# fu5ha/rayn

Measured on AMD Instinct MI355X. Metric: Mpath-samples/sec, higher is better.
Workload: dtype f32; 1 GPU; 1920x1080, 1024 spp, 8 bounces, MandelBox SDF + homogeneous volume [BASELINE configs[2]]; fma_policy=unfused (reference default build), parallelism=tiles round-robin over 1 GPU(s), build_variant=product, resolve_kernel=k_resolve_blk<128, 8>

## Files before the change

### include/rayn_hip.h

```cpp
#ifndef RAYN_HIP_H
#define RAYN_HIP_H

#include <stddef.h>
#include <stdint.h>

#ifdef __cplusplus
extern "C" {
#endif

#define RAYN_MAX_HITABLES 16
#define RAYN_MAX_MATERIALS 16
#define RAYN_MAX_LIGHTS 16
#define RAYN_FIS_TABLE_SIZE 512
#define RAYN_FILM_FLOATS_PER_PIXEL 10

typedef enum {
    RAYN_OK = 0,
    RAYN_ERR_INVALID_ARG = -1,
    RAYN_ERR_NO_DEVICE = -2,
    RAYN_ERR_HIP = -3,
    RAYN_ERR_NO_WORLD = -4,
    RAYN_ERR_OOM = -5
} rayn_status;

// ... 258 lines not shown
                            const uint32_t* d_low_object, const void* d_high_records, const uint32_t* d_high_object, float* d_out_color,
                            float* d_out_alpha, float* d_out_background, float* d_out_normal, float* d_out_weight, void* hip_stream);

typedef struct { uint32_t confidence;  } rayn_temporal_upscale_params;
int rayn_hip_temporal_upscale_device(rayn_ctx* ctx, const rayn_frame_params* p, const rayn_upscale_params* up, const rayn_temporal_params* tp,
                                     const rayn_temporal_upscale_params* sp, const rayn_camera* low_camera, const rayn_camera* prev_camera,
                                     float prev_time_start, const float* d_color, const float* d_alpha, const float* d_background,
                                     const float* d_normal, const void* d_low_records, const uint32_t* d_low_object, const void* d_high_records,
                                     const uint32_t* d_high_object, const void* d_prev_history, void* d_new_history, size_t history_bytes,
                                     float* d_out_color, float* d_out_alpha, float* d_out_background, float* d_out_normal, float* d_out_weight,
                                     void* hip_stream);

typedef struct {
    uint32_t samples;
    float radius;
    float ambient;
} rayn_preview_params;
size_t rayn_preview_scratch_bytes(uint32_t width, uint32_t height, uint32_t samples);
int rayn_hip_preview_device(rayn_ctx* ctx, const rayn_frame_params* p, const rayn_preview_params* pp, const float* d_samples,
                            const float* d_scramble, float* d_out_color, float* d_out_alpha, float* d_out_normal, float* d_out_ao,
                            void* d_out_records, uint32_t* d_out_object, void* d_scratch, size_t scratch_bytes, void* hip_stream);

typedef struct {
    float depth_tolerance;
} rayn_interpolate_params;
typedef struct {
    const float* d_color;
    const float* d_alpha;
    const float* d_background;
    const float* d_normal;
    const void* d_records;
    const uint32_t* d_object;
    const rayn_camera* camera;
    float time_start;
} rayn_interpolate_key;
int rayn_hip_interpolate_device(rayn_ctx* ctx, const rayn_frame_params* p, const rayn_interpolate_params* ip, const rayn_interpolate_key* key_a,
                                const rayn_interpolate_key* key_b, const void* d_gbuffer_records, const uint32_t* d_gbuffer_object,
                                float* d_out_color, float* d_out_alpha, float* d_out_background, float* d_out_normal, uint32_t* d_out_source,
                                void* hip_stream);

size_t rayn_png_stream_bound(uint32_t width, uint32_t height, uint32_t bpp);
size_t rayn_png_scratch_bytes(uint32_t width, uint32_t height, uint32_t bpp);
int rayn_hip_png_encode_device(rayn_ctx* ctx, uint32_t width, uint32_t height, uint32_t bpp, const uint8_t* d_img, void* d_out, size_t out_bytes,
                               void* d_scratch, size_t scratch_bytes, void* hip_stream);

size_t rayn_png_scratch_bytes_lz77(uint32_t width, uint32_t height, uint32_t bpp);
int rayn_hip_png_encode_lz77_device(rayn_ctx* ctx, uint32_t width, uint32_t height, uint32_t bpp, const uint8_t* d_img, void* d_out, size_t out_bytes,
                                    void* d_scratch, size_t scratch_bytes, void* hip_stream);
size_t rayn_deflate_stream_bound(size_t n);
size_t rayn_deflate_scratch_bytes(size_t n);
int rayn_hip_deflate_lz77_device(rayn_ctx* ctx, const void* d_data, size_t n, uint32_t stride, void* d_out, size_t out_bytes, void* d_scratch,
                                 size_t scratch_bytes, void* hip_stream);

size_t rayn_exr_stream_bound(uint32_t width, uint32_t height, uint32_t n_channels, const uint32_t* layout);
size_t rayn_exr_scratch_bytes(uint32_t width, uint32_t height, uint32_t n_channels, const uint32_t* layout, uint32_t matches);
int rayn_hip_exr_encode_device(rayn_ctx* ctx, uint32_t width, uint32_t height, uint32_t n_channels, const void* const* d_planes,
                               const uint32_t* layout, uint32_t matches, void* d_out, size_t out_bytes, void* d_scratch, size_t scratch_bytes,
                               void* hip_stream);

size_t rayn_jpeg_scan_bound(uint32_t width, uint32_t height, uint32_t bpp, uint32_t subsampling, uint32_t restart_interval);
size_t rayn_jpeg_scratch_bytes(uint32_t width, uint32_t height, uint32_t bpp, uint32_t subsampling, uint32_t restart_interval);
int rayn_jpeg_quant_table(uint32_t quality, uint32_t which, uint8_t* out);
int rayn_jpeg_huffman_table(uint32_t which, uint8_t* bits, uint8_t* vals, uint32_t n);
int rayn_hip_jpeg_encode_device(rayn_ctx* ctx, uint32_t width, uint32_t height, uint32_t bpp, uint32_t quality, uint32_t subsampling,
                                uint32_t restart_interval, const uint8_t* d_img, void* d_out, size_t out_bytes, void* d_scratch,
                                size_t scratch_bytes, void* hip_stream);

uint32_t rayn_sets_1d(uint32_t max_bounces, uint32_t volume_marches);
uint32_t rayn_sets_2d(uint32_t max_bounces, uint32_t volume_marches);
int rayn_build_rd_tables(uint32_t spp, uint32_t sets_1d, uint32_t sets_2d, uint64_t frame,
                         float* samples_1d, float* samples_2d);
int rayn_build_scramble(uint32_t width, uint32_t height, float* scramble);
enum { RAYN_FILTER_BLACKMAN_HARRIS = 0, RAYN_FILTER_BOX = 1, RAYN_FILTER_MITCHELL = 2, RAYN_FILTER_LANCZOS = 3 };
int rayn_build_fis_table(uint32_t filter_kind, float radius, float* table512);
int rayn_build_fis_table_ex(uint32_t filter_kind, float radius, float param0, float param1,
                            float* table512);
uint32_t rayn_tile_count(uint32_t width, uint32_t height, uint32_t tile_w, uint32_t tile_h);

int rayn_hip_set_profiling(rayn_ctx* ctx, int timing, int count_evals);
int rayn_hip_get_eval_counts(const rayn_ctx* ctx, uint64_t out[3]);
int rayn_hip_get_sdf_iterations(const rayn_ctx* ctx, uint64_t out[3]);
int rayn_hip_get_elision_counts(const rayn_ctx* ctx, uint64_t out[3]);
int rayn_hip_get_stage_slots(const rayn_ctx* ctx, uint64_t out[2]);
int rayn_hip_set_workers(rayn_ctx* ctx, int n_workers, uint64_t min_paths);
int rayn_hip_set_batch_paths(rayn_ctx* ctx, uint64_t paths);
int rayn_hip_set_cold_bytes(rayn_ctx* ctx, uint64_t bytes);
int rayn_hip_fma_policy(void);
int rayn_hip_set_fma_policy(rayn_ctx* ctx, int policy);
size_t rayn_hip_sizeof(int which);
const char* rayn_hip_build_variant(void);

int rayn_hip_set_tile_subset(rayn_ctx* ctx, const uint32_t* tiles, uint32_t n);

int rayn_hip_set_trace_tile(rayn_ctx* ctx, int tile_index);
int64_t rayn_hip_get_trace(const rayn_ctx* ctx, uint32_t* out, uint64_t cap_records);

int rayn_hip_probe_huffman(rayn_ctx* ctx, uint32_t n_symbols, uint32_t n_sets, const uint32_t* counts,
                           uint32_t* out_clen, uint32_t* out_tab);
int rayn_hip_probe_jpeg_transform(rayn_ctx* ctx, uint32_t width, uint32_t height, uint32_t bpp, uint32_t quality, uint32_t subsampling,
                                  const uint8_t* img, int16_t* out_coef);
int rayn_hip_probe_jpeg_entropy(rayn_ctx* ctx, uint32_t width, uint32_t height, uint32_t bpp, uint32_t subsampling, uint32_t restart_interval,
                                const int16_t* coef, uint32_t fill_byte, uint8_t* out, size_t out_bytes);
int rayn_hip_probe_shade_limits(const rayn_ctx* ctx, uint32_t* stream_blocks, uint32_t* list_ids_per_block,
                                uint32_t* setup_threads);
int rayn_hip_probe_shade(rayn_ctx* ctx, const rayn_frame_params* p, const float* samples_1d, const float* samples_2d,
                         const float* scramble, const float* fis_table, uint32_t depth, uint32_t n_slots,
                         uint32_t max_slots, uint32_t nee_cap, const uint32_t* ref, uint32_t n_pool,
                         const float* geo0, const float* geo1, const float* col0, const float* col1,
                         uint32_t sentinel, float* out_geo0, float* out_geo1, float* out_col0, float* out_col1,
                         float* out_aov, uint32_t* out_term_key, uint8_t* out_term_info,
                         uint64_t* out_alive_mask, uint8_t* out_bgrp_cnt, uint64_t* out_jobs);
int rayn_hip_probe_raygen(rayn_ctx* ctx, const rayn_frame_params* p, const float* samples_1d, uint64_t n_samples_1d,
                          const float* samples_2d, uint64_t n_samples_2d, const float* scramble, uint64_t n_scramble,
                          const float* fis_table, uint32_t n_tiles, const uint32_t* tiles, uint32_t n_pool,
                          uint32_t surplus, uint32_t sentinel, float* out_geo0, float* out_geo1, float* out_col0,
                          float* out_col1, float* out_aov, uint32_t* out_term_key, uint8_t* out_term_info,
                          uint32_t* out_q, uint32_t* out_pgrp_tile, uint32_t* out_tgb, uint32_t* out_tgc,
                          uint32_t* out_ctl, float* out_records);
int rayn_hip_probe_march_limits(const rayn_ctx* ctx, uint32_t* chunk, uint32_t* endgame_entries,
                                uint32_t* persistent_blocks, uint32_t* bulb_rays);
int rayn_hip_probe_sdf_dist(rayn_ctx* ctx, const rayn_frame_params* p, uint32_t hitable_index,
                            const float* pts_xyz, float* out, uint32_t n);
int rayn_hip_probe_sdf_dist_as(rayn_ctx* ctx, const rayn_frame_params* p, uint32_t hitable_index, int32_t sdfk,
                               uint32_t fast_div, float t0, const float* pts_xyz, float* out, uint32_t n);
int rayn_hip_probe_scene_dispatch(rayn_ctx* ctx, const rayn_frame_params* p, int32_t* out);
int rayn_hip_probe_extend(rayn_ctx* ctx, const rayn_frame_params* p, uint32_t depth,
                          const float* org_xyz, const float* dir_xyz, float* out_t,
                          uint32_t* out_obj, uint32_t n);
int rayn_hip_probe_shadow(rayn_ctx* ctx, const rayn_frame_params* p, const float* start_xyz,
                          const float* end_xyz, float* out, uint32_t n);
int rayn_hip_probe_detmath(rayn_ctx* ctx, uint32_t op, const float* a, const float* b, float* out,
                           uint32_t n);
int rayn_hip_probe_shading(rayn_ctx* ctx, const rayn_frame_params* p, uint32_t op, uint32_t index,
                           const float* in, float* out, const float* aux, uint32_t n);
int rayn_hip_probe_queue(rayn_ctx* ctx, uint32_t nclass, uint32_t n_tiles, const uint32_t* tile_groups,
                         const uint32_t* q, const uint8_t* ent_obj, const uint8_t* survive, uint32_t n_refs,
                         uint32_t cap_groups_bin, uint32_t cap_groups_repack, uint32_t max_entries,
                         uint32_t max_slots, uint32_t sentinel, uint32_t out_slots, uint32_t* out_bq,
                         uint32_t* out_qn, uint32_t* out_tile, uint32_t* out_cls_cnt,
                         uint32_t* out_cls_base, uint64_t* ctl_io);
int rayn_hip_probe_resolve(rayn_ctx* ctx, uint32_t width, uint32_t spp, uint32_t n_tiles, const uint32_t* tiles,
                           uint32_t max_tile_pixels, uint32_t n_paths, const uint8_t* term_info,
                           const uint32_t* term_key, const float* col0_rgb, const float* aov_xyz,
                           const uint32_t* aov_obj, const uint32_t* base_hist, uint32_t hist_stride,
                           uint32_t n_depths, uint32_t sentinel, uint32_t out_pixels, float* out_color,
                           float* out_alpha, float* out_background, float* out_normal);

#ifdef __cplusplus
}
#endif
#endif
```

### rayn_amd/_lib.py

```python
import ctypes as C
import os
import subprocess

from . import _abi


class RaynHipError(RuntimeError):
    pass


_CSRC = os.path.join(os.path.dirname(os.path.abspath(__file__)), "csrc")
DEFAULT_LIB_PATH = os.path.join(_CSRC, "librayn_hip.so")


def _lib_path():
    alt = os.environ.get("RAYN_HIP_LIB")
    if not alt:
        return DEFAULT_LIB_PATH
    if os.environ.get("RAYN_HIP_ALLOW_VARIANT") != "1":
        raise RaynHipError(f"RAYN_HIP_LIB={alt} is set but RAYN_HIP_ALLOW_VARIANT=1 is not: refusing to load a non-product build of librayn_hip.so")
    return alt



EXPORTS = [
    "rayn_hip_create", "rayn_hip_create_multi", "rayn_hip_device_count", "rayn_hip_table_broadcasts", "rayn_hip_destroy", "rayn_hip_last_error", "rayn_hip_upload_world", "rayn_hip_render_frame",
    "rayn_hip_render_frame_device", "rayn_hip_get_stats", "rayn_sets_1d", "rayn_sets_2d", "rayn_build_rd_tables",
    "rayn_build_scramble", "rayn_build_fis_table", "rayn_build_fis_table_ex", "rayn_tile_count", "rayn_hip_set_profiling", "rayn_hip_get_eval_counts",
    "rayn_hip_set_batch_paths", "rayn_hip_set_cold_bytes", "rayn_hip_set_workers", "rayn_hip_set_tile_subset", "rayn_hip_set_trace_tile", "rayn_hip_get_trace", "rayn_hip_fma_policy", "rayn_hip_set_fma_policy", "rayn_hip_sizeof", "rayn_hip_probe_sdf_dist",
    "rayn_hip_probe_extend", "rayn_hip_probe_shadow", "rayn_hip_probe_detmath", "rayn_hip_probe_shading", "rayn_hip_probe_queue", "rayn_hip_probe_resolve", "rayn_hip_probe_march_limits", "rayn_hip_probe_shade", "rayn_hip_probe_shade_limits", "rayn_hip_probe_raygen", "rayn_hip_probe_sdf_dist_as", "rayn_hip_probe_scene_dispatch", "rayn_hip_probe_huffman", "rayn_hip_probe_jpeg_transform", "rayn_hip_probe_jpeg_entropy", "rayn_hip_build_variant",
    "rayn_hip_get_entry_stats", "rayn_hip_get_sdf_iterations", "rayn_hip_get_elision_counts", "rayn_hip_get_stage_slots", "rayn_share_pixels", "rayn_hip_render_frame_packed_device", "rayn_hip_unpack_share_device",
    "rayn_save_to_bpp", "rayn_hip_save_to_pixels_device", "rayn_denoise_scratch_bytes", "rayn_hip_denoise_device",
    "rayn_progressive_seed", "rayn_progressive_state_bytes", "rayn_hip_progressive_reset_device", "rayn_hip_progressive_accumulate_device",
    "rayn_hip_progressive_fetch_active", "rayn_hip_progressive_tile_report",
    "rayn_denoise_variance_scratch_bytes", "rayn_hip_denoise_variance_device",
    "rayn_gbuffer_scratch_bytes", "rayn_hip_gbuffer_device", "rayn_temporal_history_bytes", "rayn_hip_temporal_accumulate_device",
    "rayn_temporal_moments_bytes", "rayn_hip_temporal_accumulate_moments_device", "rayn_hip_denoise_temporal_variance_device",
    "rayn_hip_denoise_temporal_variance_feedback_device", "rayn_hip_temporal_accumulate_resample_device",
    "rayn_display_scratch_bytes", "rayn_hip_display_pixels_device", "rayn_hip_display_color_device",
    "rayn_hip_upscale_device", "rayn_hip_temporal_upscale_device",
    "rayn_preview_scratch_bytes", "rayn_hip_preview_device",
    "rayn_hip_interpolate_device",
    "rayn_png_stream_bound", "rayn_png_scratch_bytes", "rayn_hip_png_encode_device",
    "rayn_png_scratch_bytes_lz77", "rayn_hip_png_encode_lz77_device",
    "rayn_deflate_stream_bound", "rayn_deflate_scratch_bytes", "rayn_hip_deflate_lz77_device",
    "rayn_exr_stream_bound", "rayn_exr_scratch_bytes", "rayn_hip_exr_encode_device",
    "rayn_jpeg_scan_bound", "rayn_jpeg_scratch_bytes", "rayn_jpeg_quant_table", "rayn_jpeg_huffman_table", "rayn_hip_jpeg_encode_device",
]


def build(force=False):
    if force:
        subprocess.check_call(["make", "-C", _CSRC, "clean"], stdout=subprocess.DEVNULL)
    subprocess.check_call(["make", "-C", _CSRC], stdout=subprocess.DEVNULL)


_lib = None


def lib():
    global _lib
    if _lib is None:
        LIB_PATH = _lib_path()
        if not os.path.exists(LIB_PATH):
            raise RaynHipError(f"{LIB_PATH} is missing: run `python -c 'import __graft_entry__ as g; g.build()'` "
                               "(there is no CPU fallback)")
        try:
            import torch
        except ImportError:
            pass
        L = C.CDLL(LIB_PATH)
        fp, up, vp = C.POINTER(C.c_float), C.POINTER(C.c_uint32), C.c_void_p
        L.rayn_hip_create.argtypes = [C.c_int, C.POINTER(vp)]
        L.rayn_hip_create_multi.argtypes = [C.POINTER(C.c_int), C.c_int, C.POINTER(vp)]
        L.rayn_hip_device_count.argtypes = [vp]
        L.rayn_hip_table_broadcasts.argtypes = [vp]
        L.rayn_hip_table_broadcasts.restype = C.c_uint64
        L.rayn_hip_destroy.argtypes = [vp]
        L.rayn_hip_destroy.restype = None
        L.rayn_hip_last_error.argtypes = [vp]
        L.rayn_hip_last_error.restype = C.c_char_p
        L.rayn_hip_upload_world.argtypes = [vp, C.POINTER(_abi.WorldDesc)]
        L.rayn_hip_render_frame.argtypes = [vp, C.POINTER(_abi.FrameParams), fp, fp, fp, fp, fp, fp, fp, fp]
        L.rayn_hip_render_frame_device.argtypes = [vp, C.POINTER(_abi.FrameParams)] + [vp] * 9
        L.rayn_hip_get_stats.argtypes = [vp, C.POINTER(_abi.Stats)]
        L.rayn_hip_get_entry_stats.argtypes = [vp, C.c_int, C.POINTER(_abi.Stats)]
        L.rayn_share_pixels.restype = C.c_uint64
        L.rayn_share_pixels.argtypes = [C.POINTER(_abi.FrameParams)]
        L.rayn_hip_render_frame_packed_device.argtypes = [vp, C.POINTER(_abi.FrameParams)] + [vp] * 6
        L.rayn_hip_unpack_share_device.argtypes = [vp, C.POINTER(_abi.FrameParams)] + [vp] * 6
        L.rayn_save_to_bpp.argtypes = [C.c_uint32, C.c_uint32, C.c_int]
        L.rayn_hip_save_to_pixels_device.argtypes = [vp, C.c_uint32, C.c_uint32, C.c_int, C.c_uint32, C.c_uint32] + [vp] * 6
        L.rayn_denoise_scratch_bytes.restype = C.c_size_t
        L.rayn_denoise_scratch_bytes.argtypes = [C.c_uint32, C.c_uint32]
        L.rayn_hip_denoise_device.argtypes = [vp, C.c_uint32, C.c_uint32, C.c_uint32, C.c_float, C.c_float, C.c_float] + [vp] * 5 + [C.c_size_t, vp]
        L.rayn_progressive_seed.argtypes = [C.c_uint32] * 4 + [up]
        L.rayn_progressive_state_bytes.restype = C.c_size_t
        L.rayn_progressive_state_bytes.argtypes = [C.c_uint32] * 4
        L.rayn_hip_progressive_reset_device.argtypes = [vp, C.POINTER(_abi.FrameParams), vp, C.c_size_t, vp]
        L.rayn_hip_progressive_accumulate_device.argtypes = ([vp, C.POINTER(_abi.FrameParams), C.POINTER(_abi.ProgressiveParams), up, C.c_uint32]
                                                             + [vp] * 5 + [C.c_size_t] + [vp] * 5)
        L.rayn_hip_progressive_fetch_active.restype = C.c_int64
        L.rayn_hip_progressive_fetch_active.argtypes = [vp, C.POINTER(_abi.FrameParams), vp, C.c_size_t, up, C.c_uint32,
                                                        C.POINTER(_abi.ProgressiveTotals), vp]
        L.rayn_hip_progressive_tile_report.argtypes = [vp, C.POINTER(_abi.FrameParams), vp, C.c_size_t, up, up, up, fp, vp]
        L.rayn_denoise_variance_scratch_bytes.restype = C.c_size_t
        L.rayn_denoise_variance_scratch_bytes.argtypes = [C.c_uint32, C.c_uint32]
        L.rayn_hip_denoise_variance_device.argtypes = ([vp, C.POINTER(_abi.FrameParams), C.c_uint32, C.c_float, C.c_float, C.c_float] + [vp] * 4
                                                       + [C.c_size_t, vp, vp, vp, C.c_size_t, vp])
        L.rayn_gbuffer_scratch_bytes.restype = C.c_size_t
        L.rayn_gbuffer_scratch_bytes.argtypes = [C.c_uint32, C.c_uint32]
        L.rayn_hip_gbuffer_device.argtypes = [vp, C.POINTER(_abi.FrameParams), vp, vp, vp, C.c_size_t, vp]
        L.rayn_temporal_history_bytes.restype = C.c_size_t
        L.rayn_temporal_history_bytes.argtypes = [C.c_uint32, C.c_uint32]
        L.rayn_hip_temporal_accumulate_device.argtypes = ([vp, C.POINTER(_abi.FrameParams), C.POINTER(_abi.TemporalParams), C.POINTER(_abi.Camera), C.c_float]
                                                          + [vp] * 6 + [C.c_size_t, vp, vp])
        L.rayn_temporal_moments_bytes.restype = C.c_size_t
        L.rayn_temporal_moments_bytes.argtypes = [C.c_uint32, C.c_uint32]
        L.rayn_hip_temporal_accumulate_moments_device.argtypes = ([vp, C.POINTER(_abi.FrameParams), C.POINTER(_abi.TemporalParams), C.POINTER(_abi.Camera), C.c_float]
                                                                  + [vp] * 6 + [C.c_size_t, vp, vp, C.c_size_t, vp, vp])
        L.rayn_hip_temporal_accumulate_resample_device.argtypes = ([vp, C.POINTER(_abi.FrameParams), C.POINTER(_abi.TemporalParams),
                                                                    C.POINTER(_abi.TemporalResampleParams), C.POINTER(_abi.Camera), C.c_float]
                                                                   + [vp] * 6 + [C.c_size_t, vp, vp, C.c_size_t, vp, vp])
        L.rayn_hip_denoise_temporal_variance_device.argtypes = ([vp, C.c_uint32, C.c_uint32, C.c_uint32, C.c_float, C.c_float, C.c_float] + [vp] * 5
                                                                + [C.c_size_t, vp, C.c_size_t, vp, vp, vp, C.c_size_t, vp])
        L.rayn_hip_denoise_temporal_variance_feedback_device.argtypes = ([vp, C.c_uint32, C.c_uint32, C.c_uint32, C.c_float, C.c_float, C.c_float] + [vp] * 5
                                                                         + [C.c_size_t, vp, C.c_size_t, vp, vp, vp, C.c_size_t, C.c_float, vp])
        L.rayn_display_scratch_bytes.restype = C.c_size_t
        L.rayn_display_scratch_bytes.argtypes = [C.c_uint32] * 3
        for fn in (L.rayn_hip_display_pixels_device, L.rayn_hip_display_color_device):
            fn.argtypes = [vp, C.POINTER(_abi.DisplayParams), C.c_uint32, C.c_int, C.c_uint32, C.c_uint32] + [vp] * 5 + [C.c_size_t] + [vp] * 4
        L.rayn_hip_upscale_device.argtypes = [vp, C.c_uint32, C.c_uint32, C.POINTER(_abi.UpscaleParams)] + [vp] * 14
        L.rayn_hip_temporal_upscale_device.argtypes = ([vp, C.POINTER(_abi.FrameParams), C.POINTER(_abi.UpscaleParams), C.POINTER(_abi.TemporalParams),
                                                        C.POINTER(_abi.TemporalUpscaleParams), C.POINTER(_abi.Camera), C.POINTER(_abi.Camera), C.c_float]
                                                       + [vp] * 10 + [C.c_size_t] + [vp] * 6)
        L.rayn_preview_scratch_bytes.restype = C.c_size_t
        L.rayn_preview_scratch_bytes.argtypes = [C.c_uint32] * 3
        L.rayn_hip_preview_device.argtypes = [vp, C.POINTER(_abi.FrameParams), C.POINTER(_abi.PreviewParams)] + [vp] * 9 + [C.c_size_t, vp]
        L.rayn_hip_interpolate_device.argtypes = ([vp, C.POINTER(_abi.FrameParams), C.POINTER(_abi.InterpolateParams), C.POINTER(_abi.InterpolateKey),
                                                   C.POINTER(_abi.InterpolateKey)] + [vp] * 8)
        for fn in (L.rayn_png_stream_bound, L.rayn_png_scratch_bytes, L.rayn_png_scratch_bytes_lz77):
            fn.restype = C.c_size_t
            fn.argtypes = [C.c_uint32] * 3
        for fn in (L.rayn_hip_png_encode_device, L.rayn_hip_png_encode_lz77_device):
            fn.argtypes = [vp, C.c_uint32, C.c_uint32, C.c_uint32, vp, vp, C.c_size_t, vp, C.c_size_t, vp]
        for fn in (L.rayn_deflate_stream_bound, L.rayn_deflate_scratch_bytes):
            fn.restype = C.c_size_t
            fn.argtypes = [C.c_size_t]
        L.rayn_hip_deflate_lz77_device.argtypes = [vp, vp, C.c_size_t, C.c_uint32, vp, C.c_size_t, vp, C.c_size_t, vp]
        L.rayn_exr_stream_bound.restype = C.c_size_t
        L.rayn_exr_stream_bound.argtypes = [C.c_uint32, C.c_uint32, C.c_uint32, up]
        L.rayn_exr_scratch_bytes.restype = C.c_size_t
        L.rayn_exr_scratch_bytes.argtypes = [C.c_uint32, C.c_uint32, C.c_uint32, up, C.c_uint32]
        L.rayn_hip_exr_encode_device.argtypes = [vp, C.c_uint32, C.c_uint32, C.c_uint32, C.POINTER(vp), up, C.c_uint32, vp, C.c_size_t, vp, C.c_size_t, vp]
        for fn in (L.rayn_jpeg_scan_bound, L.rayn_jpeg_scratch_bytes):
            fn.restype = C.c_size_t
            fn.argtypes = [C.c_uint32] * 5
        L.rayn_jpeg_quant_table.argtypes = [C.c_uint32, C.c_uint32, C.POINTER(C.c_uint8)]
        L.rayn_jpeg_huffman_table.argtypes = [C.c_uint32, C.POINTER(C.c_uint8), C.POINTER(C.c_uint8), C.c_uint32]
        L.rayn_hip_jpeg_encode_device.argtypes = [vp] + [C.c_uint32] * 6 + [vp, vp, C.c_size_t, vp, C.c_size_t, vp]
        L.rayn_sets_1d.restype = C.c_uint32
        L.rayn_sets_1d.argtypes = [C.c_uint32, C.c_uint32]
        L.rayn_sets_2d.restype = C.c_uint32
        L.rayn_sets_2d.argtypes = [C.c_uint32, C.c_uint32]
        L.rayn_build_rd_tables.argtypes = [C.c_uint32, C.c_uint32, C.c_uint32, C.c_uint64, fp, fp]
        L.rayn_build_scramble.argtypes = [C.c_uint32, C.c_uint32, fp]
        L.rayn_build_fis_table.argtypes = [C.c_uint32, C.c_float, fp]
        L.rayn_build_fis_table_ex.argtypes = [C.c_uint32, C.c_float, C.c_float, C.c_float, fp]
        L.rayn_tile_count.restype = C.c_uint32
        L.rayn_tile_count.argtypes = [C.c_uint32] * 4
        L.rayn_hip_set_profiling.argtypes = [vp, C.c_int, C.c_int]
        L.rayn_hip_get_eval_counts.argtypes = [vp, C.POINTER(C.c_uint64)]
        L.rayn_hip_get_sdf_iterations.argtypes = [vp, C.POINTER(C.c_uint64)]
        L.rayn_hip_get_elision_counts.argtypes = [vp, C.POINTER(C.c_uint64)]
        L.rayn_hip_get_stage_slots.argtypes = [vp, C.POINTER(C.c_uint64)]
        L.rayn_hip_set_batch_paths.argtypes = [vp, C.c_uint64]
        L.rayn_hip_set_cold_bytes.argtypes = [vp, C.c_uint64]
        L.rayn_hip_set_workers.argtypes = [vp, C.c_int, C.c_uint64]
        L.rayn_hip_set_tile_subset.argtypes = [vp, up, C.c_uint32]
        L.rayn_hip_set_trace_tile.argtypes = [vp, C.c_int]
        L.rayn_hip_get_trace.argtypes = [vp, up, C.c_uint64]
        L.rayn_hip_get_trace.restype = C.c_int64
        L.rayn_hip_set_fma_policy.argtypes = [vp, C.c_int]
        L.rayn_hip_sizeof.restype = C.c_size_t
        L.rayn_hip_sizeof.argtypes = [C.c_int]
        L.rayn_hip_probe_sdf_dist.argtypes = [vp, C.POINTER(_abi.FrameParams), C.c_uint32, fp, fp, C.c_uint32]
        L.rayn_hip_probe_extend.argtypes = [vp, C.POINTER(_abi.FrameParams), C.c_uint32, fp, fp, fp, up, C.c_uint32]
        L.rayn_hip_probe_shadow.argtypes = [vp, C.POINTER(_abi.FrameParams), fp, fp, fp, C.c_uint32]
        L.rayn_hip_probe_detmath.argtypes = [vp, C.c_uint32, fp, fp, fp, C.c_uint32]
        L.rayn_hip_probe_shading.argtypes = [vp, C.POINTER(_abi.FrameParams), C.c_uint32, C.c_uint32, fp, fp, fp, C.c_uint32]
        bp = C.POINTER(C.c_uint8)
        L.rayn_hip_probe_queue.argtypes = ([vp, C.c_uint32, C.c_uint32, up, up, bp, bp] + [C.c_uint32] * 7 + [up] * 5 + [C.POINTER(C.c_uint64)])
        L.rayn_hip_probe_resolve.argtypes = ([vp, C.c_uint32, C.c_uint32, C.c_uint32, up, C.c_uint32, C.c_uint32, bp, up, fp, fp, up, up]
                                             + [C.c_uint32] * 4 + [fp] * 4)
        L.rayn_hip_probe_march_limits.argtypes = [vp, up, up, up, up]
        L.rayn_hip_probe_shade_limits.argtypes = [vp, up, up, up]
        L.rayn_hip_probe_shade.argtypes = ([vp, C.POINTER(_abi.FrameParams), fp, fp, fp, fp] + [C.c_uint32] * 4 + [up, C.c_uint32, fp, fp, fp, fp, C.c_uint32]
                                           + [fp] * 5 + [up, bp, C.POINTER(C.c_uint64), bp, C.POINTER(C.c_uint64)])
        L.rayn_hip_probe_raygen.argtypes = ([vp, C.POINTER(_abi.FrameParams), fp, C.c_uint64, fp, C.c_uint64, fp, C.c_uint64, fp, C.c_uint32, up, C.c_uint32, C.c_uint32, C.c_uint32]
                                            + [fp] * 5 + [up, bp, up, up, up, up, up, fp])
        L.rayn_hip_probe_sdf_dist_as.argtypes = [vp, C.POINTER(_abi.FrameParams), C.c_uint32, C.c_int32, C.c_uint32, C.c_float, fp, fp, C.c_uint32]
        L.rayn_hip_probe_scene_dispatch.argtypes = [vp, C.POINTER(_abi.FrameParams), C.POINTER(C.c_int32)]
        L.rayn_hip_probe_huffman.argtypes = [vp, C.c_uint32, C.c_uint32, up, up, up]
        L.rayn_hip_probe_jpeg_transform.argtypes = [vp] + [C.c_uint32] * 5 + [vp, vp]
        L.rayn_hip_probe_jpeg_entropy.argtypes = [vp] + [C.c_uint32] * 5 + [vp, C.c_uint32, vp, C.c_size_t]
        L.rayn_hip_build_variant.restype = C.c_char_p
        L.rayn_hip_build_variant.argtypes = []
        _lib = L
    return _lib


def build_variant():
    return lib().rayn_hip_build_variant().decode()
```

### rayn_amd/context.py

```python
import ctypes as C

import numpy as np

from . import _abi
from . import progressive as _prog
from ._lib import RaynHipError, lib
from .options import JPEG_DEFAULT_RESTART


def display_scratch_bytes(width, height, levels):
    return int(lib().rayn_display_scratch_bytes(int(width), int(height), int(levels)))


def gbuffer_scratch_bytes(width, height):
    return int(lib().rayn_gbuffer_scratch_bytes(int(width), int(height)))


def temporal_history_bytes(width, height):
    return int(lib().rayn_temporal_history_bytes(int(width), int(height)))


def temporal_moments_bytes(width, height):
    return int(lib().rayn_temporal_moments_bytes(int(width), int(height)))

# ... 237 lines not shown
            first = device[0] if len(device) else 0
        else:
            rc = self._L.rayn_hip_create(device, C.byref(h))
            first = device
        if rc != 0:
            raise RaynHipError(f"rayn_hip_create(device={device}) failed with {rc} (no usable GPU?)")
        self.h = h
        self.device = first
        self.fma_policy = int(self._L.rayn_hip_fma_policy())

    def device_count(self):
        return self._L.rayn_hip_device_count(self.h)

    def _chk(self, rc):
        if rc != 0:
            raise RaynHipError(f"rayn_hip error {rc}: {self._L.rayn_hip_last_error(self.h).decode()}")

    def table_broadcasts(self):
        return int(self._L.rayn_hip_table_broadcasts(self.h))

    def last_error(self):
        return self._L.rayn_hip_last_error(self.h).decode()

    def upload_world(self, desc):
        self._chk(self._L.rayn_hip_upload_world(self.h, C.byref(desc)))

    def set_profiling(self, timing=True, count_evals=False):
        self._chk(self._L.rayn_hip_set_profiling(self.h, int(timing), int(count_evals)))

    def set_fma_policy(self, policy):
        self._chk(self._L.rayn_hip_set_fma_policy(self.h, int(policy)))
        self.fma_policy = int(policy)

    def set_workers(self, n_workers, min_paths=1 << 22):
        self._chk(self._L.rayn_hip_set_workers(self.h, int(n_workers), int(min_paths)))

    def set_tile_subset(self, tiles=None):
        arr = np.ascontiguousarray([] if tiles is None else tiles, dtype=np.uint32)
        self._chk(self._L.rayn_hip_set_tile_subset(self.h, arr.ctypes.data_as(C.POINTER(C.c_uint32)), len(arr)))

    def set_trace_tile(self, tile_index):
        self._chk(self._L.rayn_hip_set_trace_tile(self.h, int(tile_index)))

    def trace(self):
        n = self._L.rayn_hip_get_trace(self.h, None, 0)
        buf = np.zeros((max(n, 0), 6), np.uint32)
        if n > 0:
            self._L.rayn_hip_get_trace(self.h, buf.ctypes.data_as(C.POINTER(C.c_uint32)), n)
        return {k: buf[:, i].copy() for i, k in enumerate(("depth", "obj", "px", "py", "sample", "valid"))}

    def set_batch_paths(self, n):
        self._chk(self._L.rayn_hip_set_batch_paths(self.h, int(n)))

    def set_cold_bytes(self, n):
        self._chk(self._L.rayn_hip_set_cold_bytes(self.h, int(n)))

    def stats(self):
        s = _abi.Stats()
        self._chk(self._L.rayn_hip_get_stats(self.h, C.byref(s)))
        return s.as_dict()

    def entry_stats(self, entry):
        s = _abi.Stats()
        self._chk(self._L.rayn_hip_get_entry_stats(self.h, int(entry), C.byref(s)))
        return s.as_dict()

    def _counters(self, entry, names):
        out = (C.c_uint64 * len(names))()
        self._chk(entry(self.h, out))
        return dict(zip(names, out))

    def eval_counts(self):
        return self._counters(self._L.rayn_hip_get_eval_counts, ("extend", "shade_setup", "shadow"))

    def sdf_iterations(self):
        return self._counters(self._L.rayn_hip_get_sdf_iterations, ("extend", "shade_setup", "shadow"))

    def elision_counts(self):
        return self._counters(self._L.rayn_hip_get_elision_counts, ("zero_throughput_slots", "elided_shadow_jobs", "samples_out_of_bounds"))

    def stage_slots(self):
        return self._counters(self._L.rayn_hip_get_stage_slots, ("shadow_orbit", "shadow_epilogue"))

    def render_host(self, params, tables, out=None):
        s1, s2, scr, fis = tables
        n = params.width * params.height
        if out is None:
            out = {"color": np.zeros((n, 3), np.float32), "alpha": np.zeros(n, np.float32),
                   "background": np.zeros((n, 3), np.float32), "normal": np.zeros((n, 3), np.float32)}
        self._chk(self._L.rayn_hip_render_frame(self.h, C.byref(params), _fp(s1), _fp(s2), _fp(scr), _fp(fis), _fp(out["color"]),
                                                _fp(out["alpha"]), _fp(out["background"]), _fp(out["normal"])))
        h, w = params.height, params.width
        return {"color": out["color"].reshape(h, w, 3), "alpha": out["alpha"].reshape(h, w),
                "background": out["background"].reshape(h, w, 3), "normal": out["normal"].reshape(h, w, 3)}

    def probe_shade_limits(self):
        v = [C.c_uint32() for _ in range(3)]
        self._chk(self._L.rayn_hip_probe_shade_limits(self.h, *[C.byref(x) for x in v]))
        return tuple(int(x.value) for x in v)

    def probe_scene_dispatch(self, params):
        out = (C.c_int32 * (4 + _abi.MAX_HITABLES))()
        self._chk(self._L.rayn_hip_probe_scene_dispatch(self.h, C.byref(params), out))
        v = list(out)
        return {"single_sdf": v[0], "sdf_kind": v[1], "bulb": v[2], "anim_spheres": v[3], "fast_div": [x for x in v[4:] if x >= 0]}

    def probe_sdf_dist_as(self, params, hitable_index, sdfk, fast_div, pts, t0=0.0, out=None, check=True):
        pts = np.ascontiguousarray(pts, np.float32).reshape(-1, 3)
        if out is None:
            out = np.zeros(len(pts), np.float32)
        assert out.dtype == np.float32 and out.size == len(pts) and out.flags.c_contiguous
        rc = self._L.rayn_hip_probe_sdf_dist_as(self.h, C.byref(params), int(hitable_index), int(sdfk), int(fast_div), float(t0), _fp(pts), _fp(out), len(pts))
        if check:
            self._chk(rc)
        return rc, out

    RAYGEN_CTL = ("q_groups", "q_valid", "b_groups", "b_valid", "head_extend", "job_count", "head_shadow", "overflow")

    def probe_raygen(self, params, tables, tiles, n_pool, surplus=128, sentinel=0xC0FFEE5A, check=True):
        s1, s2, scr, fis = [np.ascontiguousarray(t, np.float32) for t in tables]
        tiles = np.ascontiguousarray(tiles, np.uint32).reshape(-1, 8)
        n_tiles, NP = tiles.shape[0], n_pool + surplus
        out = {k: np.zeros((NP, 4), np.float32) for k in ("geo0", "geo1", "col0", "col1", "aov")}
        out["term_key"], out["term_info"], out["q"] = np.zeros(NP, np.uint32), np.zeros(NP, np.uint8), np.zeros(NP, np.uint32)
        out["pgrp_tile"], out["tgb"], out["tgc"] = np.zeros(max(NP // 64, 1), np.uint32), np.zeros(n_tiles + 2, np.uint32), np.zeros(n_tiles + 2, np.uint32)
        ctl = np.zeros(8, np.uint32)
        spp, stride = 4 * params.samples, 8 + 12 + 8 * params.volume_marches
        recs = np.zeros((params.max_bounces + 1) * spp * stride + 64, np.float32)
        up, bp = (lambda a: a.ctypes.data_as(C.POINTER(C.c_uint32))), (lambda a: a.ctypes.data_as(C.POINTER(C.c_uint8)))
        rc = self._L.rayn_hip_probe_raygen(self.h, C.byref(params), _fp(s1), s1.size, _fp(s2), s2.size, _fp(scr), scr.size, _fp(fis), n_tiles, up(tiles), n_pool, surplus,
                                           sentinel, *[_fp(out[k]) for k in ("geo0", "geo1", "col0", "col1", "aov")], up(out["term_key"]), bp(out["term_info"]),
                                           up(out["q"]), up(out["pgrp_tile"]), up(out["tgb"]), up(out["tgc"]), up(ctl), _fp(recs))
        if check:
            self._chk(rc)
        out["ctl"] = dict(zip(self.RAYGEN_CTL, ctl.tolist()))
        out["records"], out["records_surplus"] = recs[:-64].reshape(-1, stride), recs[-64:]
        return rc, out

    def probe_shade(self, params, tables, depth, ref, geo0, geo1, col0, col1, max_slots=None, nee_cap=None, sentinel=0xC0FFEE5A, check=True):
        s1, s2, scr, fis = tables
        ref = np.ascontiguousarray(ref, np.uint32)
        recs = [np.ascontiguousarray(a, np.float32).reshape(-1, 4) for a in (geo0, geo1, col0, col1)]
        n_slots, n_pool = ref.size, recs[0].shape[0]
        assert all(a.shape[0] == n_pool for a in recs)
        out = {k: np.zeros((n_pool, 4), np.float32) for k in ("geo0", "geo1", "col0", "col1", "aov")}
        out["term_key"], out["term_info"] = np.zeros(n_pool, np.uint32), np.zeros(n_pool, np.uint8)
        groups = max(n_slots // 64, 1)
        out["alive_mask"], out["bgrp_cnt"] = np.zeros(groups, np.uint64), np.zeros(groups, np.uint8)
        jobs = np.zeros(3, np.uint64)
        up, bp, qp = (lambda a: a.ctypes.data_as(C.POINTER(C.c_uint32))), (lambda a: a.ctypes.data_as(C.POINTER(C.c_uint8))), (lambda a: a.ctypes.data_as(C.POINTER(C.c_uint64)))
        rc = self._L.rayn_hip_probe_shade(self.h, C.byref(params), _fp(s1), _fp(s2), _fp(scr), _fp(fis), depth, n_slots, n_slots if max_slots is None else max_slots,
                                          n_slots if nee_cap is None else nee_cap, up(ref), n_pool, *[_fp(a) for a in recs], sentinel,
                                          *[_fp(out[k]) for k in ("geo0", "geo1", "col0", "col1", "aov")], up(out["term_key"]), bp(out["term_info"]),
                                          qp(out["alive_mask"]), bp(out["bgrp_cnt"]), qp(jobs))
        if check:
            self._chk(rc)
        out["job_count"], out["shadow_jobs"], out["shadow_kernel"] = int(jobs[0]), int(jobs[1]), ("none", "k_shadow", "k_shadow1", "k_shadow_bulb")[int(jobs[2])]
        return rc, out

    def render_device(self, params, d_tables, d_out, stream=None):
        self._chk(self._L.rayn_hip_render_frame_device(self.h, C.byref(params), _ptr(d_tables[0]), _ptr(d_tables[1]), _ptr(d_tables[2]),
                                                       _ptr(d_tables[3]), _ptr(d_out["color"]), _ptr(d_out["alpha"]),
                                                       _ptr(d_out["background"]), _ptr(d_out["normal"]), stream_ptr(stream)))

    def render_packed(self, params, d_tables, d_packed, stream=None):
        import torch
        assert d_packed.dtype == torch.float32 and d_packed.is_contiguous() and d_packed.numel() >= 10 * share_pixels(params)
        self._chk(self._L.rayn_hip_render_frame_packed_device(self.h, C.byref(params), _ptr(d_tables[0]), _ptr(d_tables[1]), _ptr(d_tables[2]),
                                                              _ptr(d_tables[3]), _ptr(d_packed), stream_ptr(stream)))

    def unpack_share(self, params, d_packed, d_out, stream=None):
        self._chk(self._L.rayn_hip_unpack_share_device(self.h, C.byref(params), _ptr(d_packed), _ptr(d_out["color"]), _ptr(d_out["alpha"]),
                                                       _ptr(d_out["background"]), _ptr(d_out["normal"]), stream_ptr(stream)))

    def save_to_pixels(self, kind, have_mask, transparent_background, width, height, d_film, d_out, stream=None):
        import torch
        kind = getattr(kind, "value", kind)
        bpp = save_to_bpp(kind, have_mask, transparent_background)
        n = int(width) * int(height)
        if not (d_out.dtype == torch.uint8 and d_out.is_contiguous() and d_out.numel() >= n * max(bpp, 0)):
            raise ValueError(f"d_out must be a contiguous uint8 tensor of at least {n * max(bpp, 0)} bytes")
        ptrs = film_ptrs(d_film, FILM_KEYS, n, "d_film")
        self._chk(self._L.rayn_hip_save_to_pixels_device(self.h, int(kind), int(have_mask), int(bool(transparent_background)), int(width), int(height),
                                                         *ptrs, _ptr(d_out), stream_ptr(stream)))

    def png_encode_lz77(self, width, height, bpp, d_img, d_out, d_scratch=None, stream=None):
        self.png_encode(width, height, bpp, d_img, d_out, d_scratch, stream, lz77=True)

# ... 265 lines not shown
```

### rayn_amd/csrc/device_core.h

```cpp
#pragma once
#include <hip/hip_runtime.h>

#include "../../include/rayn_detmath.h"
#include "../../include/rayn_detmath_fast.h"
#include "device_scene.h"
#include "kernels.h"

#ifndef RAYN_KNS
#define RAYN_KNS rayn_p0
#endif


namespace RAYN_KNS {
using namespace rayn;

#define RD __device__ __forceinline__

RD float fmaxs(float a, float b) { return a > b ? a : b; }
RD float fmins(float a, float b) { return a < b ? a : b; }
RD float signum(float x) { return x != x ? x : __builtin_copysignf(1.0f, x); }
RD float muladd(float a, float b, float c) { return rayn_muladd(a, b, c); }
RD float lerpf(float a, float b, float t) { return a * (1.0f - t) + b * t; }

constexpr float PI_F = 3.14159265358979323846f;
// ... 63 lines not shown
RD bool in_div_window(uint32_t bits) { return bits - 0x21800000u < 0x3C000000u && (bits & 0x7FFFFFu) != 0x7FFFFFu; }
RD f3 div3_by(f3 v, float m) {
    const uint32_t ax = __float_as_uint(v.x) & 0x7FFFFFFFu, ay = __float_as_uint(v.y) & 0x7FFFFFFFu, az = __float_as_uint(v.z) & 0x7FFFFFFFu;
    const uint32_t lo = ax < ay ? (ax < az ? ax : az) : (ay < az ? ay : az);
    const uint32_t hi = ax > ay ? (ax > az ? ax : az) : (ay > az ? ay : az);
    if (lo >= 0x21800000u && hi < 0x5D800000u && in_div_window(__float_as_uint(m))) return div3_core(v, m);
    return f3{v.x / m, v.y / m, v.z / m};
}
RD f3 cross(f3 a, f3 b) {
    return f3{muladd(a.y, b.z, -a.z * b.y), muladd(a.z, b.x, -a.x * b.z), muladd(a.x, b.y, -a.y * b.x)};
}
RD f3 muladd3(f3 a, float m, f3 c) { return f3{muladd(a.x, m, c.x), muladd(a.y, m, c.y), muladd(a.z, m, c.z)}; }
RD f3 reflected(f3 v, f3 n) { return v - (2.0f * dot(v, n)) * n; }
RD float component_max(f3 a) { return fmaxs(fmaxs(a.x, a.y), a.z); }
RD bool any_nan(f3 a) { return a.x != a.x || a.y != a.y || a.z != a.z; }

struct Basis { f3 c0, c1, c2; };
RD f3 mul(const Basis& m, f3 v) { return m.c0 * v.x + m.c1 * v.y + m.c2 * v.z; }
RD Basis orthonormal_basis(f3 nor) {
    float ks = signum(nor.z);
    float ka = 1.0f / (1.0f + __builtin_fabsf(nor.z));
    float kb = -ks * nor.x * nor.y * ka;
    Basis b;
    b.c0 = f3{1.0f - nor.x * nor.x * ka, ks * kb, -ks * nor.x};
    b.c1 = f3{kb, ks - nor.y * nor.y * ka * ks, -nor.y};
    b.c2 = nor;
    return b;
}

RD void concentric_circle_map(float u0, float u1, float* ox, float* oy) {
    float a = muladd(u0, 2.0f, -1.0f);
    float b = muladd(u1, 2.0f, -1.0f);
    if (a == 0.0f && b == 0.0f) b = 0.0001f;
    float phi1 = FRAC_PI_4_F * b / a;
    float phi2 = muladd(-FRAC_PI_4_F / b, a, FRAC_PI_2_F);
    bool mask = (a * a) > (b * b);
    float r = mask ? a : b;
    float phi = mask ? phi1 : phi2;
    float s, c;
    dmf_sincosf(phi, &s, &c);
    *ox = r * c;
    *oy = r * s;
}
RD f3 cosine_weighted_in_hemisphere(float u0, float u1) {
    float x, y;
    concentric_circle_map(u0, u1, &x, &y);
    float m2 = muladd(x, x, y * y);
    float z = sqrt_rn(1.0f - fmins(m2, 1.0f));
    return f3{x, y, z};
}
RD f3 cosine_power_weighted(float u0, float u1, float power) {
    float a = dmf_powf(u0, 1.0f / (power + 1.0f));
    float a2 = a * a;
    float b = sqrt_rn(1.0f - a2);
    float s, c;
    dmf_sincosf(2.0f * u1, &s, &c);
    return f3{b * c, b * s, a};
}
RD float f_schlick(float cosv, float f0) {
    float x = 1.0f - cosv;
    float x2 = x * x;
    return f0 + (1.0f - f0) * ((x2 * x2) * x);
}


RD float sample_1d(const Tables& t, uint32_t n, uint32_t sample, float scramble, uint32_t set) {
    return dm_fractf(t.s1d[sample + n * set] + scramble);
}
RD float sample_2d(const Tables& t, uint32_t n, uint32_t dim, uint32_t sample, float scramble, uint32_t set) {
    return dm_fractf(t.s2d[dim + sample * 2 + n * 2 * set] + scramble);
}
RD float fis_sample(const float* __restrict__ inverse_cdf, float u) {
    u = 2.0f * (u - 0.5f);
    float mult = u < 0.0f ? -1.0f : 1.0f;
    u = __builtin_fabsf(u);
    u = fmaxs(u, 0.0f);
    u = fmins(u, 0.99999f);
    float idx_full = u * (float)(RAYN_FIS_TABLE_SIZE - 1);
    uint32_t idx = (uint32_t)__builtin_floorf(idx_full);
    float t = dm_fractf(idx_full);
    return mult * lerpf(inverse_cdf[idx], inverse_cdf[idx + 1], t);
}

struct EvalCtr { uint32_t n = 0, it = 0; };

__device__ __attribute__((noinline)) static float bulb_logf(float m) { return dmf_logf(m); }
struct BulbOrbit { f3 w; float m, dz; };
RD BulbOrbit bulb_begin(f3 p) { return BulbOrbit{p, p.x * p.x + p.y * p.y + p.z * p.z, 1.0f}; }
RD void bulb_step(BulbOrbit& o, f3 p) {
    const f3 w = o.w;
    const float m = o.m;
    const float m2 = m * m, m4 = m2 * m2;
    o.dz = 8.0f * sqrt_rn(m4 * m2 * m) * o.dz + 1.0f;
    const float x = w.x, x2 = x * x, x4 = x2 * x2;
    const float y = w.y, y2 = y * y, y4 = y2 * y2;
    const float z = w.z, z2 = z * z, z4 = z2 * z2;
    const float k3 = x2 + z2;
    const float k2 = rcp_sqrt_rn(k3 * k3 * k3 * k3 * k3 * k3 * k3);
    const float k1 = x4 + y4 + z4 - 6.0f * y2 * z2 - 6.0f * x2 * y2 + 2.0f * z2 * x2;
    const float k4 = x2 - y2 + z2;
    o.w.x = p.x + 64.0f * x * y * z * (x2 - z2) * k4 * (x4 - 6.0f * x2 * z2 + z4) * k1 * k2;
    o.w.y = p.y + -16.0f * y2 * k3 * k4 * k4 + k1 * k1;
    o.w.z = p.z + -8.0f * y * k4 * (x4 * x4 - 28.0f * x4 * x2 * z2 + 70.0f * x4 * z4 - 28.0f * x2 * z2 * z4 + z4 * z4) * k1 * k2;
    o.m = o.w.x * o.w.x + o.w.y * o.w.y + o.w.z * o.w.z;
}
constexpr float BULB_BAILOUT = 256.0f;
RD float bulb_finish(float m, float dz) { return 0.25f * bulb_logf(m) * sqrt_rn(m) / dz; }
RD float bulb_finish_inl(float m, float dz, const double* __restrict__ logtab) { return 0.25f * dmf_logf_t(m, logtab) * sqrt_rn(m) / dz; }
template <bool COUNT>
RD float mandelbulb_dist(f3 p, uint32_t iterations, EvalCtr& evals) {
    BulbOrbit o = bulb_begin(p);
    for (uint32_t i = 0; i < iterations; i++) {
        bulb_step(o, p);
        if (o.m > BULB_BAILOUT) { if (COUNT) evals.it -= iterations - 1u - i; break; }
    }
    return bulb_finish(o.m, o.dz);
}

RD float vmax_raw(float a, float b) {
    float r;
    asm("v_max_f32 %0, %1, %2" : "=v"(r) : "v"(a), "v"(b));
    return r;
}

RD float div_nr(float n, float d) {
    float r = __builtin_amdgcn_rcpf(d);
    const float e0 = __builtin_fmaf(-d, r, 1.0f);
    r = __builtin_fmaf(e0, r, r);
    float q = n * r;
    const float e1 = __builtin_fmaf(-d, q, n);
    q = __builtin_fmaf(e1, r, q);
    const float e2 = __builtin_fmaf(-d, q, n);
    return __builtin_fmaf(e2, r, q);
}

RD float div_short(float n, float d) {
    const float rc = __builtin_amdgcn_rcpf(d);
    const float q = n * rc;
    return __builtin_fmaf(__builtin_fmaf(-d, q, n), rc, q);
}

RD float clamp_ref(float q, float lo, float hi) {
    const float t = q > lo ? q : lo;
    return t < hi ? t : hi;
}

RD float sdf_scale(const DHitable& h, float t0) { return h.scale_vel != 0.0f ? h.scale + h.scale_vel * t0 : h.scale; }

#define RAYN_FOLD_ITER(DIV, BOX, CLAMP)                                   \
    {                                                                     \
        p.x = BOX(CLAMP(p.x, nl, l), p.x);                                \
        p.y = BOX(CLAMP(p.y, nl, l), p.y);                                \
        p.z = BOX(CLAMP(p.z, nl, l), p.z);                                \
        const float r2 = mag_sq(p);                                       \
        if (r2 < frs_eff) {  \
            const float m = DIV(frs, vmax_raw(r2, mrs_v));                \
            p.x *= m; p.y *= m; p.z *= m;                                 \
            dr *= m;                                                      \
        }                                                                 \
        p.x = muladd(p.x, s, offset.x);                                   \
        p.y = muladd(p.y, s, offset.y);                                   \
        p.z = muladd(p.z, s, offset.z);                                   \
        dr = muladd(-dr, s, 1.0f);                                        \
    }
#define RAYN_DIV_IEEE(a, b) ((a) / (b))
#define RAYN_BOX_REF(c, q) muladd(c, 2.0f, -(q))
#define RAYN_BOX_FMA(c, q) __builtin_fmaf(c, 2.0f, -(q))
#define RAYN_CLAMP_MED3(q, lo, hi) __builtin_amdgcn_fmed3f(q, lo, hi)
#define RAYN_CLAMP_REF(q, lo, hi) clamp_ref(q, lo, hi)
#define RAYN_FOLD_X4(DIV, BOX) RAYN_FOLD_ITER(DIV, BOX, RAYN_CLAMP_MED3) RAYN_FOLD_ITER(DIV, BOX, RAYN_CLAMP_MED3) RAYN_FOLD_ITER(DIV, BOX, RAYN_CLAMP_MED3) RAYN_FOLD_ITER(DIV, BOX, RAYN_CLAMP_MED3)
constexpr int SDFK_MANDELBOX_12S = 100;
template <bool COUNT, int SDFK = -1>
RD float sdf_dist(const DHitable& h, f3 p, EvalCtr& evals, float scale) {
    constexpr bool BOX12S = SDFK == SDFK_MANDELBOX_12S;
    const uint32_t kind = BOX12S ? (uint32_t)RAYN_SDF_MANDELBOX : (SDFK >= 0 ? (uint32_t)SDFK : h.sdf_kind);
    if (COUNT) { evals.n++; evals.it += kind == RAYN_SDF_SPHERE ? 0u : h.iterations; }
    if (kind == RAYN_SDF_MANDELBOX) {
        const f3 offset = p;
        float dr = 1.0f;
        const float l = h.box_l, nl = -h.box_l, s = scale;
        const float mrs = h.min_rad_sq, frs = h.fixed_rad_sq;
        const float frs_eff = mrs <= frs ? frs : -1.0f;
        float mrs_v = mrs;
        asm("" : "+v"(mrs_v));
        if (BOX12S) {
            RAYN_FOLD_X4(div_short, RAYN_BOX_FMA) RAYN_FOLD_X4(div_short, RAYN_BOX_FMA) RAYN_FOLD_X4(div_short, RAYN_BOX_FMA)
        } else if (h.fast_div == 2) {
            uint32_t i = 0;
            if (h.iterations == 12) {
                RAYN_FOLD_X4(div_short, RAYN_BOX_FMA) RAYN_FOLD_X4(div_short, RAYN_BOX_FMA) RAYN_FOLD_X4(div_short, RAYN_BOX_FMA)
                i = 12;
            }
            for (; i + 4 <= h.iterations; i += 4) { RAYN_FOLD_X4(div_short, RAYN_BOX_FMA) }
            for (; i < h.iterations; i++) RAYN_FOLD_ITER(div_short, RAYN_BOX_FMA, RAYN_CLAMP_MED3)
        } else if (h.fast_div) {
            for (uint32_t i = 0; i < h.iterations; i++) RAYN_FOLD_ITER(div_nr, RAYN_BOX_FMA, RAYN_CLAMP_MED3)
        } else {
            for (uint32_t i = 0; i < h.iterations; i++) RAYN_FOLD_ITER(RAYN_DIV_IEEE, RAYN_BOX_REF, RAYN_CLAMP_REF)
        }
        return mag(p) / __builtin_fabsf(dr);
    }
    if (kind == RAYN_SDF_MANDELBULB) return mandelbulb_dist<COUNT>(p, h.iterations, evals);
    return mag(p) - h.sdf_radius;
}
#undef RAYN_FOLD_X4
#undef RAYN_CLAMP_MED3
#undef RAYN_CLAMP_REF
#undef RAYN_FOLD_ITER
#undef RAYN_DIV_IEEE
#undef RAYN_BOX_REF
#undef RAYN_BOX_FMA

struct Thr { float k; bool constant; };
RD Thr make_thr(const DScene& sc, uint32_t depth) {
    Thr t;
    if (depth == 0) { t.k = sc.cam.half_pixel_size; t.constant = sc.cam.kind == RAYN_CAM_ORTHOGRAPHIC; }
    else { t.k = 0.0001f * 2.0f * (float)depth; t.constant = false; }
    return t;
}
RD float thr_at(const Thr& th, float t) { return th.constant ? th.k : th.k * t; }

RD f3 sphere_center(const DHitable& h, float t0) { return h.animated ? h.center + h.center_vel * t0 : h.center; }

template <bool COUNT>
RD f3 sdf_normal(const DHitable& h, f3 p, float eps, EvalCtr& evals, float sv) {
    float d1 = sdf_dist<COUNT>(h, f3{p.x + eps, p.y + -eps, p.z + -eps}, evals, sv);
    float d2 = sdf_dist<COUNT>(h, f3{p.x + -eps, p.y + -eps, p.z + eps}, evals, sv);
    float d3 = sdf_dist<COUNT>(h, f3{p.x + -eps, p.y + eps, p.z + -eps}, evals, sv);
    float d4 = sdf_dist<COUNT>(h, f3{p.x + eps, p.y + eps, p.z + eps}, evals, sv);
    f3 g = f3{1.0f * d1, -1.0f * d1, -1.0f * d1} + f3{-1.0f * d2, -1.0f * d2, 1.0f * d2} +
           f3{-1.0f * d3, 1.0f * d3, -1.0f * d3} + f3{1.0f * d4, 1.0f * d4, 1.0f * d4};
    return normalized(g);
}


RD float sphere_hit(const DHitable& h, f3 o, f3 d, float t_max, float t0) {
    f3 oc = o - sphere_center(h, t0);
    float b = dot(oc, d);
    float c = mag_sq(oc) - h.radius_sq;
    float descrim = b * b - c;
    bool desc_pos = descrim > 0.0f;
    if (!desc_pos) return 3.40282347e+38f;
    float desc_sqrt = sqrt_rn(descrim);
    float t1 = -b - desc_sqrt;
    bool t1_valid = (t1 > 0.0001f) && (t1 <= t_max) && desc_pos;
    float t2 = -b + desc_sqrt;
    bool t2_valid = (t2 > 0.0001f) && (t2 <= t_max) && desc_pos;
    bool take_t1 = (t1 < t2) && t1_valid;
    float t = take_t1 ? t1 : t2;
    return (t1_valid || t2_valid) ? t : 3.40282347e+38f;
}
RD float sphere_occluded_dir(const DHitable& h, f3 start, f3 dir, float dist, float t0) {
    f3 oc = start - sphere_center(h, t0);
    float b = dot(oc, dir);
    if (b >= 0.0f) return 1.0f;
    float c = mag_sq(oc) - h.radius_sq;
    if (c < -1e-30f) return 1.0f;
    float descrim = b * b - c;
    bool desc_pos = descrim > 0.0f;
    if (!desc_pos) return 1.0f;
    float desc_sqrt = sqrt_rn(descrim);
    float t1 = -b - desc_sqrt;
    float t2 = -b + desc_sqrt;
    float mn = fmins(t1, t2);
    bool valid = (mn > 0.001f) && (t1 <= dist) && desc_pos;
    return valid ? 0.0f : 1.0f;
}

RD void light_sample(const DLight& L, float u0, float u1, f3 p, f3* out_point, float* out_pdf) {
    f3 dir_to_light = L.pos - p;
    float dist_sq = mag_sq(dir_to_light);
    float dist = sqrt_rn(dist_sq);
    dir_to_light = div_by_mag(dir_to_light, dist);
    Basis basis = orthonormal_basis(-dir_to_light);
    float r2 = L.rad * L.rad;
    float sin_theta_max_2 = r2 / dist_sq;
    float cos_theta_max = sqrt_rn(fmaxs(0.0f, 1.0f - sin_theta_max_2));
    float cos_theta = (1.0f - u0) + u0 * cos_theta_max;
    float sin_theta = sqrt_rn(fmaxs(0.0f, 1.0f - cos_theta * cos_theta));
    float phi = u1 * TWO_PI_F;
    float ds = dist * cos_theta - sqrt_rn(fmaxs(0.0f, r2 - dist_sq * sin_theta * sin_theta));
    float cos_alpha = (dist_sq + r2 - ds * ds) / (2.0f * dist * L.rad);
    float sin_alpha = sqrt_rn(fmaxs(0.0f, 1.0f - cos_alpha * cos_alpha));
    float sin_phi, cos_phi;
    dmf_sincosf(phi, &sin_phi, &cos_phi);
    f3 offset = basis.c0 * sin_alpha * cos_phi + basis.c1 * sin_alpha * sin_phi + basis.c2 * cos_alpha;
    *out_point = L.pos + offset * L.rad;
    *out_pdf = 1.0f / (TWO_PI_F * (1.0f - cos_theta_max));
}
RD void light_sample_volume(const DLight& L, float sample, f3 ray_o, f3 ray_d, float max_distance, float* out_dist, float* out_pdf) {
    float delta = dot(L.pos - ray_o, ray_d);
    f3 closest_point = ray_o + delta * ray_d;
    float d = mag(closest_point - L.pos);
    float theta_a = dmf_atan2f(-delta, d);
    float theta_b = dmf_atan2f(max_distance - delta, d);
    float t = d * dmf_tanf(lerpf(theta_a, theta_b, sample));
    *out_dist = delta + t;
    *out_pdf = d / ((theta_b - theta_a) * muladd(d, d, t * t));
}

RD f3 bsdf_f(const DMaterial& m, f3 arg0, f3 arg1, f3 n) {
    if (m.kind == RAYN_MAT_DIELECTRIC) {
        float dt = fmaxs(0.0f, dot(arg0, n));
        float fresnel = f_schlick(dt, 0.04f);
// ... 102 lines not shown
```

### rayn_amd/csrc/device_scene.h

```cpp
#pragma once
#include <stdint.h>

#include "../../include/rayn_hip.h"

namespace rayn {

struct f3 { float x, y, z; };

struct DHitable {
    uint32_t kind, material, sdf_kind, iterations;
    f3 center; float radius_sq;
    float box_l, min_rad_sq, fixed_rad_sq, scale;
    float sdf_radius; uint32_t fast_div; uint32_t animated; uint32_t _pad;
    f3 center_vel; float scale_vel;
};
struct DMaterial { uint32_t kind, receives_light; float exponent, _pad; f3 a; float _p1; f3 b; float _p2; };
struct DLight { f3 pos; float rad; f3 emission; float _pad; };
struct DCamera {
    uint32_t kind; float half_w, half_h, full_w, full_h, half_pixel_size, aperture, _pad;
    f3 origin; float _p0; f3 at; float _p1; f3 up; float _p2; f3 focus; float _p3;
    f3 origin_vel; uint32_t animated; f3 at_vel; float _p4; f3 up_vel; float _p5; f3 focus_vel; float _p6;
};

struct DScene {
    uint32_t n_hitables, n_materials, n_lights, n_sdf;
    DHitable h[RAYN_MAX_HITABLES];
    DMaterial m[RAYN_MAX_MATERIALS];
    DLight l[RAYN_MAX_LIGHTS];
    DCamera cam;
    uint32_t has_scatter, has_extinct; float rho_s, rho_t;
    uint32_t anim_spheres;
    uint32_t sphere_mask;
    uint32_t _pad_a[2];
    uint32_t width, height, spp, max_bounces, vm, max_marches, max_vis_marches, n1, n2;
    float time_start, time_range, detail_scale, t_max, ndc_x, ndc_y;
};

struct DTile { uint32_t x0, y0, ew, eh; uint32_t pool_base, n_paths; uint32_t film_base, film_packed; };

constexpr uint32_t INVALID = 0xFFFFFFFFu;
constexpr uint32_t OBJ_NONE = 0xFFu;
constexpr uint32_t TERM_NONE = 0xFFu;

}
```

### rayn_amd/csrc/driver.h

```cpp
#pragma once
#include <hip/hip_runtime.h>
#include <stdint.h>

#include <string>
#include <utility>
#include <vector>

#include "../../include/rayn_hip.h"
#include "kernels.h"

namespace rayn {

struct ProfRec { int cls; hipEvent_t a, b; };

struct Arena {
    char* base = nullptr; size_t cap = 0, off = 0;
    template <typename T> T* take(size_t n) {
        size_t bytes = (n * sizeof(T) + 255) & ~(size_t)255;
        T* p = base ? (T*)(base + off) : nullptr;
        off += bytes;
        return p;
    }
};

struct Counters {
    unsigned long long evals[3] = {0, 0, 0};
    unsigned long long iters[3] = {0, 0, 0};
    unsigned long long elided[3] = {0, 0, 0};
    unsigned long long stage_slots[2] = {0, 0};
    void clear() { *this = Counters(); }
    Counters& operator+=(const Counters& o) {
        for (int k = 0; k < 3; k++) { evals[k] += o.evals[k]; iters[k] += o.iters[k]; elided[k] += o.elided[k]; }
        for (int k = 0; k < 2; k++) stage_slots[k] += o.stage_slots[k];
        return *this;
    }
    void decode(const unsigned long long h[16]) {
        for (int k = 0; k < 3; k++) { evals[k] = h[k]; iters[k] = h[4 + k]; }
        elided[0] = h[3]; elided[1] = h[7]; elided[2] = h[8];
        stage_slots[0] = h[12]; stage_slots[1] = h[13];
    }
};

struct Worker {
    hipStream_t stream = nullptr;
    hipStream_t own = nullptr;
    Arena arena;
    uint32_t* h_totals = nullptr;
    DCtl* h_ctl = nullptr;
    std::vector<DTile> h_tiles;
    unsigned long long* d_evals = nullptr;
    DCtl* d_ctl = nullptr;
    hipEvent_t done = nullptr;
    std::vector<ProfRec> prof;
    std::vector<hipEvent_t> event_pool;
    rayn_stats stats;
    Counters counters;
    std::string err;
    int rc = 0;
};
constexpr int MAX_WORKERS = 4;

struct Settings {
    bool have_world = false;
    rayn_world_desc world;
    bool profiling = false, counting = false;
    size_t batch_paths = (size_t)1 << 28;
    size_t two_worker_min_paths = (size_t)1 << 22;
    size_t cold_bytes = (size_t)44 << 30;
    int n_workers = 2;
    int fma_policy = 0;
};

}

struct rayn_ctx {
    int device = 0;
    hipStream_t stream = nullptr;
    std::string err;
    rayn::Settings own_cfg;
    rayn::Settings* cfg = &own_cfg;
    rayn::DScene* d_scene = nullptr;
    float4* d_rec = nullptr; size_t rec_cap = 0;
    rayn::Worker workers[rayn::MAX_WORKERS];
    hipEvent_t ev_fork = nullptr, ev_a = nullptr, ev_b = nullptr, ev_ma = nullptr, ev_mb = nullptr;
    rayn_stats stats;
    rayn::Counters counters;
    size_t small_share_paths = (size_t)1 << 27;
    uint64_t frames_rendered = 0;
    uint64_t table_broadcasts = 0;
    size_t prewarm_bytes = 0;
    float* host_stage = nullptr; size_t host_stage_cap = 0;
    rayn::Tuning tun;
    std::vector<uint32_t> tile_subset;
    std::vector<uint32_t> prog_host;
    std::vector<rayn_ctx*> peers;
    struct PeerBuf {
        float* tables = nullptr; size_t tables_cap = 0; float* packed = nullptr; size_t packed_cap = 0;
        uint64_t tab_key[10] = {0, 0, 0, 0, 0, 0, 0, 0, 0, 0}; bool tab_valid = false;
    };
    std::vector<PeerBuf> peer_bufs;
    float* gather_buf = nullptr; size_t gather_cap = 0;
    rayn::DTile* gather_tiles = nullptr; size_t gather_tiles_cap = 0;
    int budget_share = 1;
    int trace_tile = -1;
    std::vector<uint32_t> trace;
    rayn_stats entry0_stats;
    struct UnpackPlan { uint32_t key[6]; rayn::DTile* d_tiles; uint32_t n_tiles; size_t pixels; };
    std::vector<UnpackPlan> unpack_plans;
    std::vector<std::pair<std::pair<uint32_t, uint32_t>, bool>> short_div_verdicts;
};

namespace rayn {

inline int fail(rayn_ctx* c, int code, const std::string& msg) { if (c) c->err = msg; return code; }

#define HIPCHK(expr)                                                                                          \
    do {                                                                                                      \
        hipError_t e_ = (expr);                                                                               \
        if (e_ != hipSuccess) return fail(ctx, RAYN_ERR_HIP, std::string(#expr) + ": " + hipGetErrorString(e_)); \
    } while (0)

// ... 6 lines not shown
```

### rayn_amd/csrc/kernels.h

```cpp
#pragma once
#include <hip/hip_runtime.h>
#include <stdint.h>

#include "device_scene.h"

namespace rayn {

constexpr uint32_t SCAN_NC_BIN = 16;
constexpr uint32_t RESOLVE_KEY_SHIFT = 25;
static_assert(120u < (1u << (32 - RESOLVE_KEY_SHIFT)) - 1u,  "depth field of the resolve key too narrow for max_bounces <= 120 (0x7F.. is NOKEY's prefix)");
constexpr bool resolve_keys_fit(uint32_t max_tile_pixels, uint32_t spp) {
    return (unsigned long long)max_tile_pixels * spp + SCAN_NC_BIN * 3ull + 64ull < (1ull << RESOLVE_KEY_SHIFT);
}
constexpr uint32_t MAX_TILE_PIXELS = 1024, MAX_SPP_RESOLVE_BLK = 4096, MAX_BOUNCES = 120;
static_assert(resolve_keys_fit(MAX_TILE_PIXELS, MAX_SPP_RESOLVE_BLK), "k_resolve_blk's 25-bit slot offset does not cover the largest tile x spp the host accepts");
static_assert(!resolve_keys_fit(MAX_TILE_PIXELS, 8u * MAX_SPP_RESOLVE_BLK), "resolve_keys_fit must reject a segment beyond 2^25 slots");


constexpr uint32_t PROBE_SHADING_OPS = 15;
__host__ __device__ constexpr uint32_t probe_shading_in(uint32_t op) {
    return op == 0 ? 5 : op == 3 ? 3 : op == 4 ? 3 : op == 6 ? 9 : op == 7 ? 3 : op == 8 ? 11 : op == 9 ? 5 : op == 10 ? 8 : op == 13 ? 8 : op == 14 ? 7 : op >= 11 ? 1 : 2;
}
__host__ __device__ constexpr uint32_t probe_shading_out(uint32_t op) {
    return op == 0 ? 6 : op == 1 ? 2 : op == 4 ? 9 : op == 5 ? 1 : op == 8 ? 7 : op == 9 ? 4 : op == 10 ? 2 : op >= 11 ? 1 : 3;
}

struct Pool {
    float4* geo0;
    float4* geo1;
    float4* col0;
    float4* col1;
    float4* aov;
    uint32_t* term_key;
    uint8_t* term_info;
};

struct Nee {
    float* x;
    float* vtr;
    float* pdf;
    float* aux;
    uint8_t* vis;
    unsigned long long* vpicks;
    float* T;
    float* t0;
    float* nthr;
    uint8_t* flags;
    size_t cap;
    uint32_t* job_ref;
    float2* job_geo;
    size_t jobcap;
};

struct DCtl {
    uint32_t q_groups;
    uint32_t q_valid;
    uint32_t b_groups;
    uint32_t b_valid;
    uint32_t head_extend;
    uint32_t job_count;
    uint32_t head_shadow;
    uint32_t overflow;
    unsigned long long segments, shaded_slots, entries_sum, next_sum, shadow_jobs, _pad2;
};

struct QueueTables {
    uint8_t* ent_obj;
    unsigned long long* alive;
    uint8_t* grp_cnt; uint32_t *grp_base, *grp_tile;
    uint8_t* bgrp_cnt; uint32_t *bgrp_base, *bgrp_tile;
    uint32_t *ray_tgb, *ray_tgc, *bin_tgb, *bin_tgc;
    uint32_t *tile_total, *tile_valid, *tile_out_base, *tile_cls_cnt, *tile_cls_base;
};

struct ShadeHooks {
    void* user;
    void (*before_fn)(void*, int);
    void (*after_fn)(void*, int);
    void before(int i) const { if (before_fn) before_fn(user, i); }
    void after(int i) const { if (after_fn) after_fn(user, i); }
};

constexpr uint32_t CHUNK = 256;
constexpr uint32_t ENDGAME_ENTRIES = 256 * 32 * 64;

constexpr uint32_t STREAM_BLOCKS = 256 * 8;
constexpr uint32_t SCAN_ITEMS = 64;
constexpr uint32_t SHADE_SETUP_THREADS = 256;

struct Tuning {
    uint32_t persistent_blocks = 256 * 8;
    uint32_t refill_min_extend = 16;
    uint32_t refill_min_shadow = 8;
    uint32_t prefetch_min_extend = 32;
    uint32_t prefetch_min_shadow = 32;
    bool fast_path = true;
    bool sdf_templates = true;
    bool box12s = true;
    int sdf_kind = -1;
    bool bulb_path = true;
    bool bulb = false;
    uint32_t bulb_steps = 2;
    uint32_t bulb_rays = 3;
    uint32_t bulb_orbit_min = 24;
    uint32_t bulb_prefetch_min = 32;
};

enum ShadowMarchKernel { SHADOW_MARCH_GENERIC = 1 , SHADOW_MARCH_SINGLE = 2 , SHADOW_MARCH_BULB = 3  };
inline ShadowMarchKernel shadow_march_kernel(int single_sdf, const Tuning& tun) {
    if (single_sdf >= 0 && tun.fast_path) return tun.bulb ? SHADOW_MARCH_BULB : SHADOW_MARCH_SINGLE;
    return SHADOW_MARCH_GENERIC;
}

struct Tables {
    const float* __restrict__ s1d; const float* __restrict__ s2d; const float* __restrict__ fis;
    const float4* __restrict__ rec; uint32_t rec_stride;
};

}

#define RAYN_DECLARE_LAUNCHERS(NS)                                                                 \
    namespace NS {                                                                                 \
    using namespace rayn;                                                                          \
    void launch_pack_tables(hipStream_t s, Tables tab, float4* out, uint32_t spp, uint32_t depths, uint32_t n1, uint32_t n2); \
    void launch_raygen(hipStream_t s, const DScene* sc, Tables tab, const float* scramble, const DTile* tiles, const uint32_t* pgrp_tile, \
                       Pool pool, uint32_t* q, uint32_t n_pool, DCtl* ctl);                         \
    void launch_extend(hipStream_t s, bool count, const DScene* sc, uint32_t depth, const uint32_t* q, uint32_t max_entries, Pool pool, \
                       uint8_t* ent_obj, int single_sdf, DCtl* ctl, unsigned long long* evals, const Tuning& tun); \
    void launch_bin_stage(hipStream_t s, const QueueTables& T, uint32_t nclass, uint32_t n_tiles, const uint32_t* q, uint32_t max_entries, uint32_t* bq, uint32_t cap_groups, uint32_t* base_hist_row, DCtl* ctl); \
    void launch_shade(hipStream_t s, bool count, const DScene* sc, Tables tab, const float* scramble, uint32_t depth, const uint32_t* bq, \
                      uint32_t max_slots, Pool pool, Nee nee, uint32_t ns, bool has_sdf, int single_sdf, unsigned long long* alive_mask, uint8_t* bgrp_cnt, DCtl* ctl, \
                      unsigned long long* evals, ShadeHooks hooks, const Tuning& tun);              \
    void launch_repack_stage(hipStream_t s, const QueueTables& T, uint32_t n_tiles, const uint32_t* bq, uint32_t max_slots, uint32_t* qn, uint32_t cap_groups, DCtl* ctl); \
    void launch_unpack_tiles(hipStream_t s, const DTile* tiles, uint32_t n_tiles, uint32_t width, float* color, float* alpha, \
                             float* background, float* normal, const float* packed, size_t packed_pixels); \
    void launch_batch_setup(hipStream_t s, const DTile* tiles, uint32_t n_tiles, uint32_t* pgrp_tile, uint32_t* tgb, uint32_t* tgc); \
    void launch_resolve(hipStream_t s, const DScene* sc, const DTile* tiles, uint32_t n_tiles, uint32_t max_tile_pixels, uint32_t spp, Pool pool, \
                        float* out_color, float* out_alpha, float* out_background, float* out_normal, const uint32_t* base_hist, uint32_t hist_stride); \
    void launch_probe_dist(hipStream_t s, const DScene* sc, uint32_t hit_index, const float* pts, float* out, uint32_t n); \
    void launch_probe_dist_as(hipStream_t s, const DScene* sc, uint32_t hit_index, int sdfk, float t0, const float* pts, float* out, uint32_t n); \
    void launch_shadow_march(hipStream_t s, bool count, const DScene* sc, Nee nee, uint32_t max_jobs, int single_sdf, DCtl* ctl, unsigned long long* evals, const Tuning& tun); \
    void launch_probe_detmath(hipStream_t s, uint32_t op, const float* a, const float* b, float* out, uint32_t n); \
    void launch_probe_shading(hipStream_t s, const DScene* sc, uint32_t op, uint32_t index, const float* in, float* out, const float* aux, uint32_t n); \
    void launch_verify_short_div(hipStream_t s, float n, uint32_t lo_bits, uint32_t count, uint32_t* bad); \
    }
RAYN_DECLARE_LAUNCHERS(rayn_p0)
RAYN_DECLARE_LAUNCHERS(rayn_p1)

namespace rayn {
struct KernelSet {
    decltype(&rayn_p0::launch_pack_tables) pack_tables;
    decltype(&rayn_p0::launch_raygen) raygen;
    decltype(&rayn_p0::launch_extend) extend;
    decltype(&rayn_p0::launch_bin_stage) bin_stage;
    decltype(&rayn_p0::launch_shade) shade;
    decltype(&rayn_p0::launch_repack_stage) repack_stage;
    decltype(&rayn_p0::launch_batch_setup) batch_setup;
    decltype(&rayn_p0::launch_resolve) resolve;
    decltype(&rayn_p0::launch_probe_dist) probe_dist;
    decltype(&rayn_p0::launch_shadow_march) shadow_march;
    decltype(&rayn_p0::launch_probe_detmath) probe_detmath;
    decltype(&rayn_p0::launch_probe_shading) probe_shading;
    decltype(&rayn_p0::launch_probe_dist_as) probe_dist_as;
};
#define RAYN_KERNEL_SET(NS) KernelSet{&NS::launch_pack_tables, &NS::launch_raygen, &NS::launch_extend, &NS::launch_bin_stage, &NS::launch_shade, &NS::launch_repack_stage, &NS::launch_batch_setup, &NS::launch_resolve, &NS::launch_probe_dist, &NS::launch_shadow_march, &NS::launch_probe_detmath, &NS::launch_probe_shading, &NS::launch_probe_dist_as}
inline KernelSet kernel_set(int fma_policy) {
    if (fma_policy) return RAYN_KERNEL_SET(rayn_p1);
    return RAYN_KERNEL_SET(rayn_p0);
}
}
```

### rayn_amd/csrc/kernels.hip

```cpp
#include <hip/hip_runtime.h>

#include <stdlib.h>

#include <algorithm>

#include "device_core.h"
#include "kernels.h"

#if defined(__HIP_DEVICE_COMPILE__) && !defined(__gfx950__)
#error "kernels.hip is written for gfx950 (MI355X): k_resolve_blk<512, 8> / k_resolve_huge use 64 KB / 130 KB of the CU's 160 KB LDS"
#endif

namespace RAYN_KNS {

#include "march_queue.h"

__global__ void __launch_bounds__(256) k_pack_tables(Tables tab, float4* __restrict__ out, uint32_t spp, uint32_t depths, uint32_t n1, uint32_t n2) {
    const uint32_t r = blockIdx.x * blockDim.x + threadIdx.x;
    if (r >= spp * depths) return;
    const uint32_t depth = r / spp, s = r % spp;
    float* dst = (float*)(out + (size_t)r * tab.rec_stride);
    for (uint32_t k = 0; k < 8; k++) dst[k] = k < n1 ? tab.s1d[s + spp * (1 + k + depth * n1)] : 0.0f;
    for (uint32_t c = 0; c < n2; c++) dst[8 + c] = tab.s2d[(c & 1) + s * 2 + spp * 2 * (2 + (c >> 1) + depth * (n2 / 2))];
}
// ... 60 lines not shown
    const float c0 = 0.00005f * sc.detail_scale, c1 = 0.05f * sc.detail_scale;
    QueueCursor qc;
    bool has = false, first = false, nan = false;
    uint32_t ent = 0, P = 0, k = 0, id = OBJ_NONE, m = 0, sbits = 0;
    EvalCtr evals;
    f3 o = f3{0, 0, 0}, d = f3{0, 0, 0};
    float closest = 0.0f, t = 0.0f, t0 = 0.0f;
    auto advance = [&]() {
        while (k < nh) {
            const DHitable& hh = sc.h[k];
            if (hh.kind != RAYN_HITABLE_SPHERE) { first = true; return; }
            float ts = sphere_hit(hh, o, d, closest, t0);
            if (ts < closest) { closest = ts; id = k; }
            k++;
        }
        *(float2*)(&pool.geo1[P].z) = make_float2(closest, __uint_as_float((sbits & ~0xFFu) | id));
        ent_obj[ent] = (uint8_t)id;
        has = false;
    };
    bool marching = false;
    for (;;) {
        const uint64_t parked = __ballot(!marching);
        if (parked != 0 && ((uint32_t)__popcll(parked) >= REFILL_MIN || qc.exhausted)) {
            if (has && !marching) { advance(); marching = has; }
            for (;;) {
                const uint64_t need = __ballot(!has);
                if (need == 0) break;
                if (!qc.claim(head, n_entries)) break;
                const QueueSlot slot = qc.fetch(need);
                if (!has && slot.mine) {
                    ent = slot.entry;
                    P = q[ent];
                    if (P == INVALID) ent_obj[ent] = (uint8_t)OBJ_NONE;
                    else {
                        load_ray(pool, P, &o, &d, &sbits);
                        t0 = packet_time(sc, q, pool, ent);
                        closest = sc.t_max; id = OBJ_NONE; k = 0; has = true;
                        advance();
                        marching = has;
                    }
                }
            }
        }
        const uint64_t act = __ballot(marching);
        if (act == 0) {
            if (__ballot(has) == 0 && qc.exhausted) break;
            continue;
        }
        const uint32_t ku = (uint32_t)__builtin_amdgcn_readlane((int)k, (int)__builtin_ctzll(act));
        const DHitable& h = sc.h[ku];
        if (marching && k == ku) {
            const f3 ol = o - sphere_center(h, t0);
            const f3 p = first ? ol : muladd3(d, t, ol);
            const float dist = sdf_dist<COUNT>(h, p, evals, sdf_scale(h, t0));
            bool done;
            if (first) { t = dist; nan = dist != dist; first = false; m = 0; done = sc.max_marches == 0; }
            else {
                const bool hit = __builtin_fabsf(dist) < fmaxs(c0, c1 * thr_at(th, t));
                const bool gt = t > closest;
                done = hit || nan || gt;
                if (!done) { t = t + dist; m++; done = m == sc.max_marches; }
            }
            if (done) {
                if (t < closest) { closest = t; id = k; }
                k++;
                marching = false;
            }
        }
    }
    flush_evals<COUNT>(evals, evals_out);
}

template <bool COUNT, int SDFK>
__global__ void __launch_bounds__(256) k_extend1(const DScene* __restrict__ scp, uint32_t depth, uint32_t ks, const uint32_t* __restrict__ q,
                                                  DCtl* __restrict__ ctl, Pool pool, uint8_t* __restrict__ ent_obj,
                                                  uint32_t PREFETCH_MIN, unsigned long long* __restrict__ evals_out) {
    const DScene& sc = *scp;
    const uint32_t n_entries = ctl->q_groups << 6;
    uint32_t* const head = &ctl->head_extend;
    const Thr th = make_thr(sc, depth);
    const uint32_t nh = sc.n_hitables, max_marches = sc.max_marches;
    const DHitable h = sc.h[ks];
    const float c0 = 0.00005f * sc.detail_scale, c1 = 0.05f * sc.detail_scale;
    QueueCursor qc;
    uint64_t cm = 0, nm = 0, nanm = 0;
    uint32_t c_P = 0, c_ent = 0, c_ids = 0, e = 0;
    EvalCtr evals;
    f3 o = f3{0, 0, 0}, d = f3{0, 0, 0};
    f3 pt = f3{0, 0, 0};
    float c_pre = 0.0f, c_post = 0.0f, t = 0.0f;
    float c_scale = h.scale, n_scale = h.scale;
    uint32_t n_P = 0, n_ent = 0, n_ids = 0;
    f3 n_o = f3{0, 0, 0}, n_d = f3{0, 0, 0};
    float n_pre = 0.0f, n_post = 0.0f;
    for (;;) {
        const uint64_t lack = ~nm, idle = ~(cm | nm);
        if (!qc.exhausted && (qc.endgame ? idle != 0 : ((uint32_t)__popcll(lack) >= PREFETCH_MIN || (uint32_t)__popcll(idle) >= 4u))) {
            for (;;) {
                const uint64_t need = qc.endgame ? ~(nm | cm) : ~nm;
                if (need == 0) break;
                if (!qc.claim(head, n_entries, ENDGAME_ENTRIES)) break;
                const QueueSlot slot = qc.fetch(need);
                const uint64_t take = need & __builtin_amdgcn_ballot_w64(slot.mine);
                if (lane_of(take)) {
                    n_ent = slot.entry;
                    n_P = q[n_ent];
                    if (n_P == INVALID) ent_obj[n_ent] = (uint8_t)OBJ_NONE;
                    else {
                        load_ray(pool, n_P, &n_o, &n_d);
                        const float t0 = packet_time(sc, q, pool, n_ent);
                        float closest = sc.t_max;
                        uint32_t id = OBJ_NONE, idp = OBJ_NONE;
                        fold_spheres(sc, 0, ks, n_o, n_d, t0, closest, id);
                        n_pre = closest;
                        fold_spheres(sc, ks + 1, nh, n_o, n_d, t0, closest, idp);
                        n_post = closest;
                        n_ids = id | (idp << 8);
                        n_o = n_o - sphere_center(h, t0);
                        n_scale = sdf_scale(h, t0);
                    }
                }
                nm |= take & __builtin_amdgcn_ballot_w64(n_P != INVALID);
            }
        }
        const uint64_t fm = nm & ~cm;
        if (lane_of(fm)) {
            o = n_o; d = n_d; c_pre = n_pre; c_post = n_post; c_ids = n_ids; c_P = n_P; c_ent = n_ent; e = 0;
            c_scale = n_scale;
            pt = n_o;
        }
        cm |= fm; nm &= ~fm;
        if (cm == 0) {
            if (qc.exhausted) break;
            continue;
        }
        float dist = 0.0f;
        if (!COUNT) dist = sdf_dist<COUNT, SDFK>(h, pt, evals, c_scale);
        else if (lane_of(cm)) dist = sdf_dist<COUNT, SDFK>(h, pt, evals, c_scale);
        const uint64_t stop = (__builtin_amdgcn_ballot_w64(__builtin_fabsf(dist) < fmaxs(c0, c1 * thr_at(th, t))) | __builtin_amdgcn_ballot_w64(t > c_pre) | nanm) & ~fm;
        nanm = (nanm & ~fm) | (__builtin_amdgcn_ballot_w64(dist != dist) & fm);
        const float ts = t + dist;
        const float tg = lane_of(fm) ? dist : ts;
        t = lane_of(stop) ? t : tg;
        e++;
        const uint64_t fin = (stop | __builtin_amdgcn_ballot_w64(e == max_marches + 1u)) & cm;
        if (lane_of(fin)) {
            float closest = c_pre;
            uint32_t id = c_ids & 0xFFu;
            if (t < closest) { closest = t; id = ks; }
            const uint32_t idp = c_ids >> 8;
            if (idp != OBJ_NONE && c_post < closest) { closest = c_post; id = idp; }
            pool.geo1[c_P].z = closest;
            ((uint8_t*)&pool.geo1[c_P].w)[0] = (uint8_t)id;
            ent_obj[c_ent] = (uint8_t)id;
        }
        cm &= ~fin;
        pt = muladd3(d, t, o);
    }
    flush_evals<COUNT>(evals, evals_out);
}

constexpr uint32_t QUEUE_UNROLL = 8;

RD uint32_t quad_total(uint32_t n) {
    n += (uint32_t)__builtin_amdgcn_update_dpp(0, (int)n, 0xB1, 0xF, 0xF, true);
    n += (uint32_t)__builtin_amdgcn_update_dpp(0, (int)n, 0x4E, 0xF, 0xF, true);
    return n;
}
RD uint32_t count_eq4(uint32_t v, uint32_t pat) {
    const uint32_t x = v ^ pat;
    return (uint32_t)__popc(~(((x & 0x7F7F7F7Fu) + 0x7F7F7F7Fu) | x | 0x7F7F7F7Fu));
}
__global__ void __launch_bounds__(256) k_group_hist(uint32_t nclass, const uint8_t* __restrict__ ent_obj, const DCtl* __restrict__ ctl,
                                                     uint8_t* __restrict__ grp_cnt) {
    const uint32_t n_q = ctl->q_groups << 2;
    const uint4* __restrict__ obj16 = (const uint4*)ent_obj;
    const uint32_t stride = gridDim.x * blockDim.x;
    constexpr uint32_t HIST_UNROLL = 2;
    for (uint32_t i0 = blockIdx.x * blockDim.x + threadIdx.x; i0 < n_q; i0 += stride * HIST_UNROLL) {
        uint4 v[HIST_UNROLL];
#pragma unroll
        for (uint32_t u = 0; u < HIST_UNROLL; u++) { const uint32_t i = i0 + u * stride; v[u] = i < n_q ? obj16[i] : make_uint4(~0u, ~0u, ~0u, ~0u); }
#pragma unroll
        for (uint32_t u = 0; u < HIST_UNROLL; u++) {
            const uint32_t i = i0 + u * stride;
            uint32_t acc[4] = {0u, 0u, 0u, 0u};
            for (uint32_t c = 0; c < nclass; c++) {
                const uint32_t pat = c * 0x01010101u;
                const uint32_t n = quad_total(count_eq4(v[u].x, pat) + count_eq4(v[u].y, pat) + count_eq4(v[u].z, pat) + count_eq4(v[u].w, pat));
                const uint32_t sh = n << (8u * (c & 3u));
                if ((c >> 2) == 0) acc[0] |= sh; else if ((c >> 2) == 1) acc[1] |= sh; else if ((c >> 2) == 2) acc[2] |= sh; else acc[3] |= sh;
            }
            if (i < n_q && (threadIdx.x & 3u) == 3u) *(uint4*)(grp_cnt + (size_t)(i >> 2) * SCAN_NC_BIN) = make_uint4(acc[0], acc[1], acc[2], acc[3]);
        }
    }
}
__global__ void __launch_bounds__(256) k_scan_tile(uint32_t nclass, uint32_t stride, uint32_t pad, const uint8_t* __restrict__ grp_cnt,
                                                    const uint32_t* __restrict__ tile_grp_begin, const uint32_t* __restrict__ tile_grp_count,
                                                    uint32_t* __restrict__ grp_base, uint32_t* __restrict__ grp_tile,
                                                    uint32_t* __restrict__ tile_total, uint32_t* __restrict__ tile_valid,
                                                    uint32_t* __restrict__ tile_cls_cnt, const DCtl* __restrict__ ctl) {
    if (ctl->overflow) return;
    __shared__ uint32_t s_tot[SCAN_NC_BIN];
    const uint32_t k = blockIdx.x;
    const uint32_t gb = tile_grp_begin[k], gc = tile_grp_count[k];
    const uint32_t lane = lane_id(), wave = threadIdx.x >> 6;
    for (uint32_t gi = threadIdx.x; gi < gc; gi += 256) grp_tile[gb + gi] = k;
    for (uint32_t c = wave; c < nclass; c += 4) {
        uint32_t run = 0;
        for (uint32_t base = 0; base < gc; base += 64 * QUEUE_UNROLL) {
            uint32_t v[QUEUE_UNROLL];
#pragma unroll
            for (uint32_t u = 0; u < QUEUE_UNROLL; u++) {
                const uint32_t gi = base + u * 64 + lane;
                v[u] = gi < gc ? grp_cnt[(size_t)(gb + gi) * stride + c] : 0u;
            }
#pragma unroll
            for (uint32_t u = 0; u < QUEUE_UNROLL; u++) {
                const uint32_t gi = base + u * 64 + lane;
                uint32_t inc = v[u];
#pragma unroll
                for (int off = 1; off < 64; off <<= 1) {
                    const uint32_t n = __shfl_up(inc, off);
                    if (lane >= (uint32_t)off) inc += n;
                }
                if (gi < gc) grp_base[(size_t)(gb + gi) * stride + c] = run + inc - v[u];
                run += (uint32_t)__builtin_amdgcn_readlane((int)inc, 63);
            }
// ... 1356 lines not shown
```

### rayn_amd/csrc/march_queue.h

```cpp
#pragma once

RD uint32_t lane_id() { return threadIdx.x & 63u; }
RD bool lane_of(uint64_t mask) { return __builtin_amdgcn_inverse_ballot_w64(mask); }
RD uint32_t mbcnt(uint64_t mask) {
    return __builtin_amdgcn_mbcnt_hi((uint32_t)(mask >> 32), __builtin_amdgcn_mbcnt_lo((uint32_t)mask, 0u));
}

struct QueueSlot { bool mine; uint32_t entry; };
struct QueueCursor {
    uint32_t cur = 0, end = 0;
    bool exhausted = false;
    bool endgame = false;
    RD uint32_t take_chunk(uint32_t* head, uint32_t n) {
        uint32_t base = 0;
        if (lane_id() == 0) base = atomicAdd(head, CHUNK);
        base = __builtin_amdgcn_readfirstlane(base);
        if (base >= n) return 0;
        cur = base; end = min(base + CHUNK, n);
        return n - base;
    }
    RD bool claim(uint32_t* head, uint32_t n, uint32_t endgame_entries = 0) {
        if (cur == end && !exhausted) {
            const uint32_t left = take_chunk(head, n);
            if (left == 0) exhausted = true; else endgame = left < endgame_entries;
        }
        return !exhausted;
    }
    RD QueueSlot fetch(uint64_t need) {
        const uint32_t rank = mbcnt(need), avail = end - cur;
        const QueueSlot slot = QueueSlot{rank < avail, cur + rank};
        cur += min((uint32_t)__popcll(need), avail);
        return slot;
    }
};

RD void store_job(float2* __restrict__ job_geo, size_t idx, f3 a, f3 b) {
    job_geo[3 * idx] = make_float2(a.x, a.y);
    job_geo[3 * idx + 1] = make_float2(a.z, b.x);
    job_geo[3 * idx + 2] = make_float2(b.y, b.z);
}
RD void load_job(const Nee& nee, const DScene& sc, uint32_t ref, f3* a, f3* b, float* t0) {
    const float2 j0 = nee.job_geo[3 * (size_t)ref], j1 = nee.job_geo[3 * (size_t)ref + 1], j2 = nee.job_geo[3 * (size_t)ref + 2];
    *a = f3{j0.x, j0.y, j1.x}; *b = f3{j1.y, j2.x, j2.y};
    *t0 = sc.anim_spheres ? nee.t0[ref % (uint32_t)nee.cap] : 0.0f;
}

RD void sdf_segment(const DHitable& h, f3 a, f3 b, float t0, f3* start, f3* dir, float* max_dist) {
    const f3 origin = sphere_center(h, t0);
    *start = a - origin;
    const f3 d = (b - origin) - *start;
    *max_dist = mag(d);
    *dir = div_by_mag(d, *max_dist);
}

constexpr uint32_t MS_FIRST = 1u << 16, MS_NAN = 1u << 17, MS_COUNT = 0xFFFFu;
RD int occluded_step(uint32_t& ms, float& t, float dist, float max_dist, float c0, float c1, uint32_t max_vis) {
    bool nan = (ms & MS_NAN) != 0;
    int res = -1;
    if (ms & MS_FIRST) {
        t = dist; nan = dist != dist; ms = nan ? MS_NAN : 0u;
        if (max_vis == 0) res = ((dist < 0.0001f) && !((dist > max_dist) || nan)) ? 0 : 1;
        else if ((t > max_dist) || nan) res = 1;
    } else {
        if (__builtin_fabsf(dist) < fmaxs(c0, c1 * t)) res = 0;
        else {
            t = t + dist; ms++;
            if ((ms & MS_COUNT) == max_vis || (t > max_dist) || nan) res = 1;
        }
    }
    return res;
}

RD void fold_spheres(const DScene& sc, uint32_t k_begin, uint32_t k_end, f3 o, f3 d, float t0, float& closest, uint32_t& id) {
    for (uint32_t k = k_begin; k < k_end; k++) {
        const float ts = sphere_hit(sc.h[k], o, d, closest, t0);
        if (ts < closest) { closest = ts; id = k; }
    }
}
RD void load_ray(const Pool& pool, uint32_t P, f3* o, f3* d) {
    const float4 g0 = pool.geo0[P];
    const float2 g1 = *(const float2*)(&pool.geo1[P].x);
    *o = f3{g0.x, g0.y, g0.z}; *d = f3{g0.w, g1.x, g1.y};
}
RD void load_ray(const Pool& pool, uint32_t P, f3* o, f3* d, uint32_t* sbits) {
    const float4 g0 = pool.geo0[P], g1 = pool.geo1[P];
    *o = f3{g0.x, g0.y, g0.z}; *d = f3{g0.w, g1.x, g1.y}; *sbits = __float_as_uint(g1.w);
}

template <bool COUNT>
RD void flush_evals(const EvalCtr& evals, unsigned long long* __restrict__ evals_out) {
    if (COUNT && evals.n) { atomicAdd(evals_out, (unsigned long long)evals.n); atomicAdd(evals_out + 4, (unsigned long long)evals.it); }
}
```

### rayn_amd/csrc/probes.hip

```cpp
#include <hip/hip_runtime.h>
#include <string.h>

#include <algorithm>
#include <string>
#include <vector>

#include "driver.h"
#include "frame_layout.h"
#include "jpeg.h"
#include "png_device.h"

using namespace rayn;

namespace {
struct DevBuf {
    void* p = nullptr;
    ~DevBuf() { if (p) (void)hipFree(p); }
    hipError_t alloc(size_t bytes) { return hipMalloc(&p, bytes ? bytes : 4); }
    template <typename T> T* as() const { return (T*)p; }
};
struct ProbeArena : Arena {
    ~ProbeArena() { if (base) (void)hipFree(base); }
    template <typename F> hipError_t alloc(F carve) {
        Arena dry; carve(dry);
// ... 21 lines not shown
static int probe_common(rayn_ctx* ctx, const rayn_frame_params* p, DScene* out_hs = nullptr) {
    int rc = validate(ctx, p);
    if (rc) return rc;
    HIPCHK(hipSetDevice(ctx->device));
    DScene hs;
    rc = build_scene(ctx, ctx->cfg->world, *p, &hs);
    if (rc) return rc;
    HIPCHK(hipMemcpy(ctx->d_scene, &hs, sizeof hs, hipMemcpyHostToDevice));
    if (out_hs) *out_hs = hs;
    return RAYN_OK;
}
static int probe_counters(rayn_ctx* ctx, const unsigned long long* d_ev) {
    unsigned long long h[16];
    HIPCHK(hipMemcpy(h, d_ev, sizeof h, hipMemcpyDeviceToHost));
    ctx->counters.decode(h);
    return RAYN_OK;
}
static int probe_pool_out(rayn_ctx* ctx, const Pool& pool, size_t n, float* geo0, float* geo1, float* col0, float* col1, float* aov, uint32_t* term_key, uint8_t* term_info) {
    HIPCHK(hipMemcpy(geo0, pool.geo0, n * 16, hipMemcpyDeviceToHost)); HIPCHK(hipMemcpy(geo1, pool.geo1, n * 16, hipMemcpyDeviceToHost));
    HIPCHK(hipMemcpy(col0, pool.col0, n * 16, hipMemcpyDeviceToHost)); HIPCHK(hipMemcpy(col1, pool.col1, n * 16, hipMemcpyDeviceToHost));
    HIPCHK(hipMemcpy(aov, pool.aov, n * 16, hipMemcpyDeviceToHost)); HIPCHK(hipMemcpy(term_key, pool.term_key, n * 4, hipMemcpyDeviceToHost));
    HIPCHK(hipMemcpy(term_info, pool.term_info, n, hipMemcpyDeviceToHost));
    return RAYN_OK;
}
int rayn_hip_probe_sdf_dist(rayn_ctx* ctx, const rayn_frame_params* p, uint32_t hitable_index, const float* pts, float* out, uint32_t n) {
    int rc = probe_common(ctx, p);
    if (rc) return rc;
    if (hitable_index >= ctx->cfg->world.n_hitables || ctx->cfg->world.hitables[hitable_index].kind != RAYN_HITABLE_TRACED_SDF)
        return fail(ctx, RAYN_ERR_INVALID_ARG, "hitable_index does not name a TracedSDF of the uploaded world");
    if (!pts || !out) return fail(ctx, RAYN_ERR_INVALID_ARG, "null buffer");
    const KernelSet K = kernel_set(ctx->cfg->fma_policy);
    DevBuf d_in, d_out;
    HIPCHK(d_in.alloc((size_t)n * 12)); HIPCHK(d_out.alloc((size_t)n * 4));
    HIPCHK(hipMemcpy(d_in.p, pts, (size_t)n * 12, hipMemcpyHostToDevice));
    K.probe_dist(ctx->stream, ctx->d_scene, hitable_index, d_in.as<float>(), d_out.as<float>(), n);
    HIPCHK(hipStreamSynchronize(ctx->stream));
    HIPCHK(hipMemcpy(out, d_out.p, (size_t)n * 4, hipMemcpyDeviceToHost));
    return RAYN_OK;
}
int rayn_hip_probe_sdf_dist_as(rayn_ctx* ctx, const rayn_frame_params* p, uint32_t hitable_index, int32_t sdfk, uint32_t fast_div, float t0, const float* pts,
                               float* out, uint32_t n) {
    int rc = validate(ctx, p);
    if (rc) return rc;
    HIPCHK(hipSetDevice(ctx->device));
    DScene hs;
    rc = build_scene(ctx, ctx->cfg->world, *p, &hs);
    if (rc) return rc;
    if (hitable_index >= ctx->cfg->world.n_hitables || ctx->cfg->world.hitables[hitable_index].kind != RAYN_HITABLE_TRACED_SDF)
        return fail(ctx, RAYN_ERR_INVALID_ARG, "hitable_index does not name a TracedSDF of the uploaded world");
    if (!pts || !out) return fail(ctx, RAYN_ERR_INVALID_ARG, "null buffer");
    if (n == 0 || n > (1u << 26)) return fail(ctx, RAYN_ERR_INVALID_ARG, "probe size out of range");
    DHitable& h = hs.h[hitable_index];
    if (sdfk != -1 && sdfk != (int32_t)RAYN_SDF_SPHERE && sdfk != (int32_t)RAYN_SDF_MANDELBOX && sdfk != (int32_t)RAYN_SDF_MANDELBULB && sdfk != 100)
        return fail(ctx, RAYN_ERR_INVALID_ARG, "sdfk names no instantiation of sdf_dist (-1, a RAYN_SDF_* kind or 100)");
    if (sdfk >= 0 && sdfk != 100 && (uint32_t)sdfk != h.sdf_kind) return fail(ctx, RAYN_ERR_INVALID_ARG, "sdfk is not the SDF kind of the object");
    if (sdfk == 100 && (h.sdf_kind != RAYN_SDF_MANDELBOX || h.fast_div != 2u || h.iterations != 12u))
        return fail(ctx, RAYN_ERR_INVALID_ARG, "sdfk 100 needs a 12-iteration MandelBox whose short division the upload verified (fast_div 2)");
    if (fast_div > h.fast_div) return fail(ctx, RAYN_ERR_INVALID_ARG, "fast_div may only lower the object's own division arm");
    if (sdfk == 100 && fast_div != 2u) return fail(ctx, RAYN_ERR_INVALID_ARG, "sdfk 100 has the short division compiled in: fast_div must be 2");
    h.fast_div = fast_div;
    const KernelSet K = kernel_set(ctx->cfg->fma_policy);
    DevBuf d_sc, d_in, d_out;
    HIPCHK(d_sc.alloc(sizeof hs)); HIPCHK(d_in.alloc((size_t)n * 12)); HIPCHK(d_out.alloc((size_t)n * 4));
    HIPCHK(hipMemcpy(d_sc.p, &hs, sizeof hs, hipMemcpyHostToDevice));
    HIPCHK(hipMemcpy(d_in.p, pts, (size_t)n * 12, hipMemcpyHostToDevice));
    K.probe_dist_as(ctx->stream, d_sc.as<DScene>(), hitable_index, sdfk, t0, d_in.as<float>(), d_out.as<float>(), n);
    HIPCHK(hipStreamSynchronize(ctx->stream));
    HIPCHK(hipGetLastError());
    HIPCHK(hipMemcpy(out, d_out.p, (size_t)n * 4, hipMemcpyDeviceToHost));
    return RAYN_OK;
}
int rayn_hip_probe_scene_dispatch(rayn_ctx* ctx, const rayn_frame_params* p, int32_t* out) {
    int rc = validate(ctx, p);
    if (rc) return rc;
    if (!out) return fail(ctx, RAYN_ERR_INVALID_ARG, "null buffer");
    HIPCHK(hipSetDevice(ctx->device));
    DScene hs;
    rc = build_scene(ctx, ctx->cfg->world, *p, &hs);
    if (rc) return rc;
    Tuning tun;
    out[0] = scene_march_kernels(ctx, hs, *p, &tun);
    out[1] = tun.sdf_kind; out[2] = tun.bulb ? 1 : 0; out[3] = (int32_t)hs.anim_spheres;
    for (uint32_t i = 0; i < RAYN_MAX_HITABLES; i++) out[4 + i] = i < hs.n_hitables ? (int32_t)hs.h[i].fast_div : -1;
    return RAYN_OK;
}
int rayn_hip_probe_extend(rayn_ctx* ctx, const rayn_frame_params* p, uint32_t depth, const float* org, const float* dir, float* out_t,
                          uint32_t* out_obj, uint32_t n) {
    DScene hs;
    int rc = probe_common(ctx, p, &hs);
    if (rc) return rc;
    if (!org || !dir || !out_t || !out_obj) return fail(ctx, RAYN_ERR_INVALID_ARG, "null buffer");
    if (n == 0 || n > (1u << 26)) return fail(ctx, RAYN_ERR_INVALID_ARG, "probe size out of range");
    Tuning tun;
    const int single_sdf = scene_march_kernels(ctx, hs, *p, &tun);
    const KernelSet K = kernel_set(ctx->cfg->fma_policy);
    const uint32_t npad = (n + 63u) & ~63u;
    std::vector<float4> g0(n), g1(n);
    std::vector<uint32_t> q(npad, INVALID);
    uint32_t none_bits = OBJ_NONE;
    float none_f; memcpy(&none_f, &none_bits, 4);
    for (uint32_t i = 0; i < n; i++) {
        g0[i] = make_float4(org[3 * i], org[3 * i + 1], org[3 * i + 2], dir[3 * i]);
        g1[i] = make_float4(dir[3 * i + 1], dir[3 * i + 2], 0.0f, none_f);
        q[i] = i;
    }
    DCtl hc;
    memset(&hc, 0, sizeof hc);
    hc.q_groups = npad / 64; hc.q_valid = n;
    DevBuf d_g0, d_g1, d_c1, d_q, d_obj, d_ctl, d_ev;
    HIPCHK(d_g0.alloc((size_t)n * 16)); HIPCHK(d_g1.alloc((size_t)n * 16)); HIPCHK(d_c1.alloc((size_t)n * 16)); HIPCHK(d_q.alloc((size_t)npad * 4));
    HIPCHK(d_obj.alloc(npad)); HIPCHK(d_ctl.alloc(sizeof(DCtl))); HIPCHK(d_ev.alloc(128));
    HIPCHK(hipMemcpy(d_g0.p, g0.data(), (size_t)n * 16, hipMemcpyHostToDevice)); HIPCHK(hipMemcpy(d_g1.p, g1.data(), (size_t)n * 16, hipMemcpyHostToDevice));
    HIPCHK(hipMemset(d_c1.p, 0, (size_t)n * 16));
    HIPCHK(hipMemcpy(d_q.p, q.data(), (size_t)npad * 4, hipMemcpyHostToDevice)); HIPCHK(hipMemset(d_obj.p, 0xEE, npad));
    HIPCHK(hipMemcpy(d_ctl.p, &hc, sizeof hc, hipMemcpyHostToDevice)); HIPCHK(hipMemset(d_ev.p, 0, 128));
    Pool pool;
    memset(&pool, 0, sizeof pool);
    pool.geo0 = d_g0.as<float4>(); pool.geo1 = d_g1.as<float4>(); pool.col1 = d_c1.as<float4>();
    const bool count = ctx->cfg->counting;
    K.extend(ctx->stream, count, ctx->d_scene, depth, d_q.as<uint32_t>(), npad, pool, d_obj.as<uint8_t>(), single_sdf, d_ctl.as<DCtl>(), d_ev.as<unsigned long long>(), tun);
    HIPCHK(hipStreamSynchronize(ctx->stream));
    HIPCHK(hipGetLastError());
    if (count) { rc = probe_counters(ctx, d_ev.as<unsigned long long>()); if (rc) return rc; }
    std::vector<uint8_t> obj(npad);
    HIPCHK(hipMemcpy(g1.data(), d_g1.p, (size_t)n * 16, hipMemcpyDeviceToHost)); HIPCHK(hipMemcpy(obj.data(), d_obj.p, npad, hipMemcpyDeviceToHost));
    for (uint32_t i = 0; i < n; i++) {
        uint32_t bits; memcpy(&bits, &g1[i].w, 4);
        if ((bits & 0xFFu) != obj[i]) return fail(ctx, RAYN_ERR_HIP, "internal: the pool's hit object and the per-entry object byte disagree");
        out_t[i] = g1[i].z;
        out_obj[i] = obj[i] == OBJ_NONE ? INVALID : obj[i];
    }
    for (uint32_t i = n; i < npad; i++) if (obj[i] != OBJ_NONE) return fail(ctx, RAYN_ERR_HIP, "internal: a padding entry of the queue was not marked empty");
    return RAYN_OK;
}
int rayn_hip_probe_shadow(rayn_ctx* ctx, const rayn_frame_params* p, const float* start, const float* end, float* out, uint32_t n) {
    DScene hs;
    int rc = probe_common(ctx, p, &hs);
    if (rc) return rc;
    if (!start || !end || !out) return fail(ctx, RAYN_ERR_INVALID_ARG, "null buffer");
    if (n == 0 || n > (1u << 26)) return fail(ctx, RAYN_ERR_INVALID_ARG, "probe size out of range");
    if (hs.n_sdf == 0) return fail(ctx, RAYN_ERR_INVALID_ARG, "the uploaded world holds no TracedSDF: nothing to march");
    Tuning tun;
    const int single_sdf = scene_march_kernels(ctx, hs, *p, &tun);
    const KernelSet K = kernel_set(ctx->cfg->fma_policy);
    std::vector<float2> geo(3 * (size_t)n);
    std::vector<uint32_t> ref(n);
    for (uint32_t i = 0; i < n; i++) {
        geo[3 * (size_t)i] = make_float2(start[3 * i], start[3 * i + 1]);
        geo[3 * (size_t)i + 1] = make_float2(start[3 * i + 2], end[3 * i]);
        geo[3 * (size_t)i + 2] = make_float2(end[3 * i + 1], end[3 * i + 2]);
        ref[i] = i;
    }
    DCtl hc;
    memset(&hc, 0, sizeof hc);
    hc.job_count = n;
    DevBuf d_geo, d_ref, d_vis, d_t0, d_ctl, d_ev;
    HIPCHK(d_geo.alloc((size_t)n * 24)); HIPCHK(d_ref.alloc((size_t)n * 4)); HIPCHK(d_vis.alloc(n)); HIPCHK(d_t0.alloc((size_t)n * 4));
    HIPCHK(d_ctl.alloc(sizeof(DCtl))); HIPCHK(d_ev.alloc(128));
    HIPCHK(hipMemcpy(d_geo.p, geo.data(), (size_t)n * 24, hipMemcpyHostToDevice)); HIPCHK(hipMemcpy(d_ref.p, ref.data(), (size_t)n * 4, hipMemcpyHostToDevice));
    HIPCHK(hipMemset(d_vis.p, 2, n));
    HIPCHK(hipMemset(d_t0.p, 0, (size_t)n * 4)); HIPCHK(hipMemcpy(d_ctl.p, &hc, sizeof hc, hipMemcpyHostToDevice)); HIPCHK(hipMemset(d_ev.p, 0, 128));
    Nee nee;
    memset(&nee, 0, sizeof nee);
    nee.vis = d_vis.as<uint8_t>(); nee.t0 = d_t0.as<float>(); nee.cap = n; nee.job_ref = d_ref.as<uint32_t>(); nee.job_geo = d_geo.as<float2>(); nee.jobcap = n;
    const bool count = ctx->cfg->counting;
    K.shadow_march(ctx->stream, count, ctx->d_scene, nee, n, single_sdf, d_ctl.as<DCtl>(), d_ev.as<unsigned long long>(), tun);
// ... 531 lines not shown
```

### rayn_amd/csrc/rayn_hip.hip

```cpp
#include <hip/hip_runtime.h>
#include <stdio.h>
#include <stdlib.h>
#include <string.h>

#include <algorithm>
#include <cmath>
#include <string>
#include <thread>
#include <vector>

#include "../../include/rayn_detmath.h"
#include "../../include/rayn_hip.h"
#include "driver.h"
#include "frame_layout.h"
#include "tiles.h"
#include "save_to.h"
#include "display.h"
#include "temporal_upscale.h"
#include "upscale.h"
#include "denoise.h"
#include "denoise_variance.h"
#include "post_checks.h"
#include "preview.h"
#include "interpolate.h"
#include "jpeg.h"
#include "png.h"
#include "exr.h"
#include "progressive.h"
#include "temporal.h"

using namespace rayn;

namespace {

enum ProfClass { PC_RAYGEN = 0, PC_EXTEND, PC_BIN, PC_SHADE, PC_COMPACT, PC_RESOLVE, PC_SHADOW, PC_FINISH, PC_COUNT };

int wfail(Worker* w, int code, const std::string& msg) { w->err = msg; w->rc = code; return code; }

#define WCHK(expr)                                                                                            \
    do {                                                                                                      \
        hipError_t e_ = (expr);                                                                               \
        if (e_ != hipSuccess) return wfail(w, RAYN_ERR_HIP, std::string(#expr) + ": " + hipGetErrorString(e_)); \
    } while (0)

f3 to3(rayn_vec3 v) { return f3{v.x, v.y, v.z}; }

uint32_t f32_bits(float f) { uint32_t u; memcpy(&u, &f, 4); return u; }

bool short_div_is_exact(rayn_ctx* ctx, float mrs, float frs) {
    if (!(mrs > 0.0f) || !(mrs < frs)) return false;
    const std::pair<uint32_t, uint32_t> key(f32_bits(mrs), f32_bits(frs));
    for (const auto& e : ctx->short_div_verdicts) if (e.first == key) return e.second;
    bool ok = false;
    uint32_t* d_bad = nullptr;
    uint32_t bad = 1;
    if (hipSetDevice(ctx->device) == hipSuccess && hipMalloc((void**)&d_bad, 4) == hipSuccess) {
        if (hipMemsetAsync(d_bad, 0, 4, ctx->stream) == hipSuccess) {
            rayn_p0::launch_verify_short_div(ctx->stream, frs, key.first, key.second - key.first, d_bad);
            if (hipMemcpyAsync(&bad, d_bad, 4, hipMemcpyDeviceToHost, ctx->stream) == hipSuccess && hipStreamSynchronize(ctx->stream) == hipSuccess)
                ok = bad == 0;
        }
        hipFree(d_bad);
    }
    ctx->short_div_verdicts.emplace_back(key, ok);
    return ok;
}

}

namespace rayn {

bool build_camera(const rayn_camera& c, DCamera* out) {
    memset(out, 0, sizeof *out);
    DCamera& dc = *out;
    dc.kind = c.kind; dc.origin = to3(c.origin); dc.at = to3(c.at); dc.up = to3(c.up); dc.focus = to3(c.focus); dc.aperture = c.aperture;
    dc.animated = c.animated & 15u; dc.origin_vel = to3(c.origin_vel); dc.at_vel = to3(c.at_vel); dc.up_vel = to3(c.up_vel); dc.focus_vel = to3(c.focus_vel);
    if (c.kind == RAYN_CAM_ORTHOGRAPHIC) {
        float aspect = c.res_w / c.res_h;
        float sx = c.vfov_or_size * aspect, sy = c.vfov_or_size;
        float pixel_size = c.vfov_or_size / c.res_h;
        dc.half_w = sx / 2.0f; dc.half_h = sy / 2.0f; dc.full_w = sx; dc.full_h = sy;
        dc.half_pixel_size = pixel_size / 2.0f;
    } else if (c.kind == RAYN_CAM_PINHOLE || c.kind == RAYN_CAM_THIN_LENS) {
        float theta = c.vfov_or_size * 3.14159265358979323846f / 180.0f;
        float half_height = dm_tanf(theta / 2.0f);
        float aspect = c.res_w / c.res_h;
        float half_width = aspect * half_height;
        dc.half_pixel_size = half_height / c.res_h;
        dc.half_w = half_width; dc.half_h = half_height; dc.full_w = half_width; dc.full_h = half_height;
    } else return false;
    return true;
}

int build_scene(rayn_ctx* ctx, const rayn_world_desc& w, const rayn_frame_params& p, DScene* out) {
    DScene& s = *out;
    memset(&s, 0, sizeof s);
    if (w.n_hitables > RAYN_MAX_HITABLES || w.n_materials > RAYN_MAX_MATERIALS || w.n_lights > RAYN_MAX_LIGHTS)
        return fail(ctx, RAYN_ERR_INVALID_ARG, "world exceeds fixed capacities");
    s.n_hitables = w.n_hitables; s.n_materials = w.n_materials; s.n_lights = w.n_lights;
    for (uint32_t i = 0; i < w.n_hitables; i++) {
        const rayn_hitable& h = w.hitables[i];
        DHitable& d = s.h[i];
        if (h.material >= w.n_materials) return fail(ctx, RAYN_ERR_INVALID_ARG, "hitable references a missing material");
        d.kind = h.kind; d.material = h.material; d.sdf_kind = h.sdf_kind; d.iterations = h.iterations;
        d.center = to3(h.center);
        d.animated = h.animated ? 1u : 0u; d.center_vel = to3(h.center_vel);
        d.scale_vel = (h.kind == RAYN_HITABLE_TRACED_SDF && h.sdf_kind == RAYN_SDF_MANDELBOX) ? h.scale_vel : 0.0f;
        if (d.animated || d.scale_vel != 0.0f) s.anim_spheres = 1;
        d.radius_sq = h.radius * h.radius;
        d.box_l = h.box_side;
        d.min_rad_sq = h.min_radius * h.min_radius;
        d.fixed_rad_sq = h.fixed_radius * h.fixed_radius;
        d.scale = h.scale;
        d.sdf_radius = h.sdf_radius;
        {
            const float lo = 8.6736174e-19f , hi = 1.1529215e18f ;
            const float bs = h.box_side < 0.0f ? -h.box_side : h.box_side;
            d.fast_div = (d.min_rad_sq >= lo && d.min_rad_sq <= hi && d.fixed_rad_sq >= lo && d.fixed_rad_sq <= hi && bs <= hi) ? 1u : 0u;
            if (!(h.box_side >= 0.0f) || std::signbit(h.box_side)) d.fast_div = 0u;
            if (d.fast_div && h.kind == RAYN_HITABLE_TRACED_SDF && h.sdf_kind == RAYN_SDF_MANDELBOX && short_div_is_exact(ctx, d.min_rad_sq, d.fixed_rad_sq))
                d.fast_div = 2u;
        }
        if (h.kind == RAYN_HITABLE_TRACED_SDF) {
            s.n_sdf++;
            if (h.sdf_kind != RAYN_SDF_SPHERE && h.sdf_kind != RAYN_SDF_MANDELBOX && h.sdf_kind != RAYN_SDF_MANDELBULB) return fail(ctx, RAYN_ERR_INVALID_ARG, "unknown sdf_kind");
        } else if (h.kind == RAYN_HITABLE_SPHERE) s.sphere_mask |= 1u << i;
        else return fail(ctx, RAYN_ERR_INVALID_ARG, "unknown hitable kind");
    }
    for (uint32_t i = 0; i < w.n_materials; i++) {
        const rayn_material& m = w.materials[i];
        DMaterial& d = s.m[i];
        if (m.kind > RAYN_MAT_EMISSIVE) return fail(ctx, RAYN_ERR_INVALID_ARG, "unknown material kind");
        d.kind = m.kind; d.a = to3(m.a); d.b = to3(m.b); d.exponent = m.exponent;
        d.receives_light = (m.kind == RAYN_MAT_SKY || m.kind == RAYN_MAT_EMISSIVE) ? 0u : 1u;
    }
    for (uint32_t i = 0; i < w.n_lights; i++) {
        s.l[i].pos = to3(w.lights[i].pos); s.l[i].rad = w.lights[i].rad; s.l[i].emission = to3(w.lights[i].emission);
    }
    if (!build_camera(w.camera, &s.cam)) return fail(ctx, RAYN_ERR_INVALID_ARG, "unknown camera kind");
    s.has_scatter = w.has_scattering; s.has_extinct = w.has_extinction; s.rho_s = w.coeff_scattering; s.rho_t = w.coeff_extinction;
    s.width = p.width; s.height = p.height; s.spp = p.samples * 4; s.max_bounces = p.max_bounces; s.vm = p.volume_marches;
    s.max_marches = p.max_marches; s.max_vis_marches = p.max_vis_marches;
    s.n1 = 3 + p.volume_marches; s.n2 = 12 + 8 * p.volume_marches;
    s.time_start = p.time_start; s.time_range = p.time_end - p.time_start;
    s.detail_scale = p.sdf_detail_scale; s.t_max = p.world_radius * 2.0f;
    s.ndc_x = 1.0f / (float)p.width; s.ndc_y = 1.0f / (float)p.height;
    return RAYN_OK;
}

int scene_march_kernels(const rayn_ctx* ctx, const DScene& hs, const rayn_frame_params& p, Tuning* tun) {
    int single_sdf = -1;
    if (hs.n_sdf == 1) for (uint32_t i = 0; i < hs.n_hitables; i++) if (hs.h[i].kind == RAYN_HITABLE_TRACED_SDF) single_sdf = (int)i;
    *tun = ctx->tun;
    tun->sdf_kind = single_sdf >= 0 && ctx->tun.sdf_templates ? (int)hs.h[single_sdf].sdf_kind : -1;
    if (tun->sdf_kind == (int)RAYN_SDF_MANDELBOX && ctx->tun.box12s && hs.h[single_sdf].fast_div == 2u && hs.h[single_sdf].iterations == 12u) tun->sdf_kind = 100;
    tun->bulb = ctx->tun.bulb_path && single_sdf >= 0 && hs.h[single_sdf].sdf_kind == RAYN_SDF_MANDELBULB && hs.h[single_sdf].iterations >= 1 &&
                p.max_marches < 0xFFFFu && p.max_vis_marches < 0xFFFFu;
    return single_sdf;
}

int validate(rayn_ctx* ctx, const rayn_frame_params* p) {
    if (!ctx) return RAYN_ERR_INVALID_ARG;
    if (!p) return fail(ctx, RAYN_ERR_INVALID_ARG, "null frame params");
    if (!ctx->cfg->have_world) return fail(ctx, RAYN_ERR_NO_WORLD, "rayn_hip_upload_world has not been called");
    if (!p->width || !p->height || !p->samples || !p->tile_w || !p->tile_h) return fail(ctx, RAYN_ERR_INVALID_ARG, "zero-sized frame, tile or sample count");
    if (p->volume_marches < 2 || p->volume_marches > 4) return fail(ctx, RAYN_ERR_INVALID_ARG, "volume_marches must be in [2,4] (samples_1d[3],[4] are indexed, src/integrator.rs:138,175)");
    if (p->max_bounces > MAX_BOUNCES) return fail(ctx, RAYN_ERR_INVALID_ARG, "max_bounces > 120 does not fit the 7-bit depth field of the termination record");
    if (p->samples > 4096) return fail(ctx, RAYN_ERR_INVALID_ARG, "spp > 16384 unsupported (the film resolve sorts a pixel's samples in the registers of one 1024-thread block)");
    if ((uint64_t)p->tile_w * (uint64_t)p->tile_h > MAX_TILE_PIXELS) return fail(ctx, RAYN_ERR_INVALID_ARG, "tile larger than 1024 pixels unsupported");
    if ((uint64_t)p->width * (uint64_t)p->height >= ((uint64_t)1 << 31)) return fail(ctx, RAYN_ERR_INVALID_ARG, "film larger than 2^31 pixels unsupported (32-bit pixel indices)");
    return RAYN_OK;
}

}

namespace {

hipEvent_t get_event(Worker* w) {
    if (!w->event_pool.empty()) { hipEvent_t e = w->event_pool.back(); w->event_pool.pop_back(); return e; }
    hipEvent_t e;
    if (hipEventCreate(&e) != hipSuccess) return nullptr;
    return e;
}

int ensure_worker(rayn_ctx* ctx, Worker* w, bool own_stream) {
    bool ok = hipSetDevice(ctx->device) == hipSuccess;
    if (ok && !w->d_ctl)
        ok = hipMalloc((void**)&w->d_evals, 128) == hipSuccess && hipMalloc((void**)&w->d_ctl, sizeof(DCtl)) == hipSuccess &&
             hipHostMalloc((void**)&w->h_totals, 16) == hipSuccess && hipHostMalloc((void**)&w->h_ctl, sizeof(DCtl)) == hipSuccess &&
             hipEventCreateWithFlags(&w->done, hipEventDisableTiming) == hipSuccess;
    if (ok && own_stream && !w->own) ok = hipStreamCreateWithFlags(&w->own, hipStreamNonBlocking) == hipSuccess;
    return ok ? RAYN_OK : fail(ctx, RAYN_ERR_HIP, std::string("worker resources: ") + hipGetErrorString(hipGetLastError()));
}

struct Timed {
    Worker* w; bool on; hipStream_t s; int cls; hipEvent_t a = nullptr, b = nullptr;
    Timed(Worker* w_, bool on_, int cl) : w(w_), on(on_), s(w_->stream), cls(cl) {
        if (on) { a = get_event(w); b = get_event(w); if (a) (void)hipEventRecord(a, s); }
    }
    ~Timed() {
        if (on && a && b) { (void)hipEventRecord(b, s); w->prof.push_back(ProfRec{cls, a, b}); }
    }
};

void add(rayn_stats& a, const rayn_stats& b) {
    a.paths += b.paths; a.segments += b.segments; a.shaded_slots += b.shaded_slots; a.tiles += b.tiles; a.batches += b.batches;
    a.launches_extend += b.launches_extend; a.launches_shade += b.launches_shade; a.shadow_jobs += b.shadow_jobs;
    a.queue_bytes_bin += b.queue_bytes_bin; a.queue_bytes_compact += b.queue_bytes_compact;
    a.ms_raygen += b.ms_raygen; a.ms_extend += b.ms_extend; a.ms_bin += b.ms_bin; a.ms_shade += b.ms_shade; a.ms_compact += b.ms_compact;
    a.ms_resolve += b.ms_resolve; a.ms_shadow += b.ms_shadow; a.ms_finish += b.ms_finish;
}

void collect_profile(rayn_ctx* ctx) {
    double ms[PC_COUNT] = {0};
    for (Worker& w : ctx->workers) {
        for (auto& r : w.prof) {
            float t = 0;
            if (hipEventElapsedTime(&t, r.a, r.b) == hipSuccess) ms[r.cls] += t;
            w.event_pool.push_back(r.a);
            w.event_pool.push_back(r.b);
        }
        w.prof.clear();
    }
    ctx->stats.ms_raygen = ms[PC_RAYGEN]; ctx->stats.ms_extend = ms[PC_EXTEND]; ctx->stats.ms_bin = ms[PC_BIN];
    ctx->stats.ms_shade = ms[PC_SHADE]; ctx->stats.ms_compact = ms[PC_COMPACT]; ctx->stats.ms_resolve = ms[PC_RESOLVE];
    ctx->stats.ms_shadow = ms[PC_SHADOW]; ctx->stats.ms_finish = ms[PC_FINISH];
}

struct BatchTile { uint32_t tile_index; DTile d; };
// ... 371 lines not shown
            if (he == hipSuccess) he = hipMemcpyPeerAsync(t2, c->device, d_s2, ctx->device, n2 * 4, c->stream);
            if (he == hipSuccess) he = hipMemcpyPeerAsync(tscr, c->device, d_scr, ctx->device, npx * 4, c->stream);
            if (he == hipSuccess) he = hipMemcpyPeerAsync(tfis, c->device, d_fis, ctx->device, RAYN_FIS_TABLE_SIZE * 4, c->stream);
            if (he == hipSuccess) { memcpy(B.tab_key, key, sizeof key); B.tab_valid = true; ctx->table_broadcasts++; }
        }
        if (he != hipSuccess) return bail(RAYN_ERR_HIP, std::string("table broadcast: ") + hipGetErrorString(he));
        r = render_device(c, p, t1, t2, tscr, tfis, t, c->stream);
        if (r) return bail(r, c->err);
        if (px) {
            he = hipMemcpyPeerAsync(ctx->gather_buf + gather_off[e] * 10, ctx->device, B.packed, c->device, px * 40, c->stream);
            if (he == hipSuccess) he = hipStreamSynchronize(c->stream);
            if (he != hipSuccess) return bail(RAYN_ERR_HIP, std::string("film gather: ") + hipGetErrorString(he));
        }
    };
    {
        std::vector<std::thread> threads;
        for (size_t e = 1; e < N; e++) threads.emplace_back(run_entry, e);
        run_entry(0);
        for (auto& t : threads) t.join();
    }
    HIPCHK(hipSetDevice(ctx->device));
    for (size_t e = 0; e < N; e++) if (rcs[e]) return fail(ctx, rcs[e], "device entry " + std::to_string(e) + ": " + errs[e]);
    size_t t_off = 0;
    for (size_t e = 1; e < N; e++) {
        const std::vector<DTile>& pack = mine[e].d;
        if (pack.empty()) continue;
        HIPCHK(hipMemcpyAsync(ctx->gather_tiles + t_off, pack.data(), pack.size() * sizeof(DTile), hipMemcpyHostToDevice, stream));
        rayn_p0::launch_unpack_tiles(stream, ctx->gather_tiles + t_off, (uint32_t)pack.size(), p->width, out.color, out.alpha, out.bg, out.normal,
                                     ctx->gather_buf + gather_off[e] * 10, mine[e].pixels);
        t_off += pack.size();
    }
    HIPCHK(hipEventRecord(ctx->ev_mb, stream));
    HIPCHK(hipStreamSynchronize(stream));
    ctx->entry0_stats = ctx->stats;
    rayn_stats total = ctx->stats;
    for (rayn_ctx* c : ctx->peers) { add(total, c->stats); ctx->counters += c->counters; }
    float ms = 0;
    (void)hipEventElapsedTime(&ms, ctx->ev_ma, ctx->ev_mb);
    total.ms_total = ms;
    ctx->stats = total;
    return RAYN_OK;
}

int render_any(rayn_ctx* ctx, const rayn_frame_params* p, const float* d_s1, const float* d_s2, const float* d_scr, const float* d_fis,
               const RenderTarget& out, hipStream_t stream) {
    if (ctx && !ctx->peers.empty()) return render_multi(ctx, p, d_s1, d_s2, d_scr, d_fis, out, stream);
    return render_device(ctx, p, d_s1, d_s2, d_scr, d_fis, out, stream);
}

}

extern "C" {

int rayn_hip_create(int device, rayn_ctx** out) {
    if (!out) return RAYN_ERR_INVALID_ARG;
    *out = nullptr;
    int n = 0;
    if (hipGetDeviceCount(&n) != hipSuccess || n <= 0) return RAYN_ERR_NO_DEVICE;
    if (device < 0 || device >= n) return RAYN_ERR_INVALID_ARG;
    rayn_ctx* ctx = new rayn_ctx();
    ctx->device = device;
    memset(&ctx->stats, 0, sizeof ctx->stats);
    bool ok = hipSetDevice(device) == hipSuccess && hipStreamCreate(&ctx->stream) == hipSuccess &&
              hipMalloc((void**)&ctx->d_scene, sizeof(DScene)) == hipSuccess && hipEventCreate(&ctx->ev_a) == hipSuccess &&
              hipEventCreate(&ctx->ev_b) == hipSuccess && hipEventCreateWithFlags(&ctx->ev_fork, hipEventDisableTiming) == hipSuccess;
    if (!ok) { rayn_hip_destroy(ctx); return RAYN_ERR_HIP; }
    if (const char* sw = getenv("RAYN_HIP_ENV_TUNING")) if (atoi(sw) != 0) {
        if (const char* e = getenv("RAYN_HIP_WORKERS")) ctx->cfg->n_workers = atoi(e);
        if (const char* e = getenv("RAYN_HIP_WORKER_MIN_PATHS")) ctx->cfg->two_worker_min_paths = (size_t)atoll(e);
        if (const char* e = getenv("RAYN_HIP_BATCH_PATHS")) { long long v = atoll(e); if (v >= 4096) ctx->cfg->batch_paths = (size_t)v; }
        if (const char* e = getenv("RAYN_HIP_COLD_BYTES")) { long long v = atoll(e); ctx->cfg->cold_bytes = v > 0 ? (size_t)v : 0; }
        if (const char* e = getenv("RAYN_HIP_PROFILE")) ctx->cfg->profiling = atoi(e) != 0;
        if (const char* e = getenv("RAYN_HIP_REFILL_EXTEND")) ctx->tun.refill_min_extend = (uint32_t)std::max(1, atoi(e));
        if (const char* e = getenv("RAYN_HIP_REFILL_SHADOW")) ctx->tun.refill_min_shadow = (uint32_t)std::max(1, atoi(e));
        if (const char* e = getenv("RAYN_HIP_PREFETCH_EXTEND")) ctx->tun.prefetch_min_extend = (uint32_t)std::max(1, atoi(e));
        if (const char* e = getenv("RAYN_HIP_PREFETCH_SHADOW")) ctx->tun.prefetch_min_shadow = (uint32_t)std::max(1, atoi(e));
        if (const char* e = getenv("RAYN_HIP_FAST_PATH")) ctx->tun.fast_path = atoi(e) != 0;
        if (const char* e = getenv("RAYN_HIP_PERSISTENT_BLOCKS")) ctx->tun.persistent_blocks = (uint32_t)std::max(1, atoi(e));
        if (const char* e = getenv("RAYN_HIP_SDF_TEMPLATES")) ctx->tun.sdf_templates = atoi(e) != 0;
        if (const char* e = getenv("RAYN_HIP_BULB_PATH")) ctx->tun.bulb_path = atoi(e) != 0;
        if (const char* e = getenv("RAYN_HIP_BULB_STEPS")) ctx->tun.bulb_steps = atoi(e) == 2 ? 2u : 1u;
        if (const char* e = getenv("RAYN_HIP_BULB_ORBIT_MIN")) ctx->tun.bulb_orbit_min = (uint32_t)std::max(0, atoi(e));
        if (const char* e = getenv("RAYN_HIP_BOX12S")) ctx->tun.box12s = atoi(e) != 0;
        if (const char* e = getenv("RAYN_HIP_BULB_RAYS")) ctx->tun.bulb_rays = (uint32_t)std::min(4, std::max(2, atoi(e)));
        if (const char* e = getenv("RAYN_HIP_BULB_PREFETCH")) ctx->tun.bulb_prefetch_min = (uint32_t)std::max(1, atoi(e));
    }
    *out = ctx;
    return RAYN_OK;
}

int rayn_hip_create_multi(const int* devices, int n_devices, rayn_ctx** out) {
    if (!out) return RAYN_ERR_INVALID_ARG;
    *out = nullptr;
    if (!devices || n_devices < 1 || n_devices > 64) return RAYN_ERR_INVALID_ARG;
    rayn_ctx* ctx = nullptr;
    int rc = rayn_hip_create(devices[0], &ctx);
    if (rc) return rc;
    for (int i = 1; i < n_devices; i++) {
        rayn_ctx* c = nullptr;
        rc = rayn_hip_create(devices[i], &c);
        if (rc) { rayn_hip_destroy(ctx); return rc; }
        c->cfg = &ctx->own_cfg;
        ctx->peers.push_back(c);
        if (devices[i] != devices[0]) {
            int can = 0;
            if (hipDeviceCanAccessPeer(&can, devices[0], devices[i]) == hipSuccess && can) {
                (void)hipSetDevice(devices[0]); (void)hipDeviceEnablePeerAccess(devices[i], 0);
                (void)hipSetDevice(devices[i]); (void)hipDeviceEnablePeerAccess(devices[0], 0);
                (void)hipGetLastError();
            }
        }
    }
    ctx->peer_bufs.resize(ctx->peers.size());
    for (int i = 0; i < n_devices; i++) {
        int share = 0;
        for (int j = 0; j < n_devices; j++) share += devices[j] == devices[i];
        (i == 0 ? ctx : ctx->peers[i - 1])->budget_share = share;
    }
    (void)hipSetDevice(devices[0]);
    *out = ctx;
    return RAYN_OK;
}

int rayn_hip_device_count(const rayn_ctx* ctx) { return ctx ? (int)(1 + ctx->peers.size()) : 0; }
uint64_t rayn_hip_table_broadcasts(const rayn_ctx* ctx) { return ctx ? ctx->table_broadcasts : 0; }

void rayn_hip_destroy(rayn_ctx* ctx) {
    if (!ctx) return;
    for (size_t i = 0; i < ctx->peers.size(); i++) {
        rayn_ctx* c = ctx->peers[i];
        (void)hipSetDevice(c->device);
        if (i < ctx->peer_bufs.size()) {
            rayn_ctx::PeerBuf& B = ctx->peer_bufs[i];
            if (B.tables) (void)hipFree(B.tables);
            if (B.packed) (void)hipFree(B.packed);
        }
        rayn_hip_destroy(c);
    }
    ctx->peers.clear();
    (void)hipSetDevice(ctx->device);
    if (ctx->gather_buf) (void)hipFree(ctx->gather_buf);
    if (ctx->gather_tiles) (void)hipFree(ctx->gather_tiles);
    for (auto& up : ctx->unpack_plans) if (up.d_tiles) (void)hipFree(up.d_tiles);
    ctx->unpack_plans.clear();
    if (ctx->stream) (void)hipStreamSynchronize(ctx->stream);
    for (Worker& w : ctx->workers) {
        if (w.own) (void)hipStreamSynchronize(w.own);
        for (auto e : w.event_pool) (void)hipEventDestroy(e);
        if (w.d_ctl) (void)hipFree(w.d_ctl);
        if (w.arena.base) (void)hipFree(w.arena.base);
        if (w.d_evals) (void)hipFree(w.d_evals);
        if (w.h_totals) (void)hipHostFree(w.h_totals);
        if (w.h_ctl) (void)hipHostFree(w.h_ctl);
        if (w.done) (void)hipEventDestroy(w.done);
        if (w.own) (void)hipStreamDestroy(w.own);
    }
    if (ctx->d_rec) (void)hipFree(ctx->d_rec);
    if (ctx->host_stage) (void)hipFree(ctx->host_stage);
    if (ctx->d_scene) (void)hipFree(ctx->d_scene);
    if (ctx->ev_a) (void)hipEventDestroy(ctx->ev_a);
    if (ctx->ev_b) (void)hipEventDestroy(ctx->ev_b);
    if (ctx->ev_ma) (void)hipEventDestroy(ctx->ev_ma);
    if (ctx->ev_mb) (void)hipEventDestroy(ctx->ev_mb);
    if (ctx->ev_fork) (void)hipEventDestroy(ctx->ev_fork);
    if (ctx->stream) (void)hipStreamDestroy(ctx->stream);
    delete ctx;
// ... 460 lines not shown
    if (out_totals) {
        out_totals->active_tiles = h[0];
        memcpy(&out_totals->max_e, &h[1], 4);
        out_totals->outlier_pixels = (uint64_t)h[2] | ((uint64_t)h[3] << 32);
    }
    if (out_tiles) memcpy(out_tiles, h + 4, (size_t)h[0] * 4u);
    return (int64_t)h[0];
}

int rayn_hip_progressive_tile_report(rayn_ctx* ctx, const rayn_frame_params* p, const void* d_state, size_t state_bytes, uint32_t* out_epochs,
                                     uint32_t* out_retired, uint32_t* out_outliers, float* out_max_e, void* hip_stream) {
    ProgLayout L;
    hipStream_t s;
    if (int rc = post_enter(ctx, progressive_geometry(p, d_state, state_bytes, &L), hip_stream, &s)) return rc;
    ctx->prog_host.resize((size_t)L.n_tiles * 4u);
    HIPCHK(hipMemcpyAsync(ctx->prog_host.data(), (const char*)d_state + L.off_records, (size_t)L.n_tiles * 16u, hipMemcpyDeviceToHost, s));
    HIPCHK(hipStreamSynchronize(s));
    for (uint32_t k = 0; k < L.n_tiles; k++) {
        const uint32_t* r = ctx->prog_host.data() + (size_t)k * 4u;
        if (out_epochs) out_epochs[k] = r[0];
        if (out_retired) out_retired[k] = r[1];
        if (out_outliers) out_outliers[k] = r[2];
        if (out_max_e) memcpy(&out_max_e[k], &r[3], 4);
    }
    return RAYN_OK;
}

int rayn_hip_get_entry_stats(const rayn_ctx* ctx, int entry, rayn_stats* out) {
    if (!ctx || !out || entry < 0 || entry > (int)ctx->peers.size()) return RAYN_ERR_INVALID_ARG;
    if (ctx->peers.empty()) *out = ctx->stats;
    else *out = entry == 0 ? ctx->entry0_stats : ctx->peers[(size_t)entry - 1]->stats;
    return RAYN_OK;
}

int rayn_hip_render_frame(rayn_ctx* ctx, const rayn_frame_params* p, const float* samples_1d, const float* samples_2d, const float* scramble,
                          const float* fis_table, float* out_color, float* out_alpha, float* out_background, float* out_normal) {
    int rc = check_frame_args(ctx, p, samples_1d, samples_2d, scramble, fis_table, RenderTarget{out_color, out_alpha, out_background, out_normal});
    if (rc) return rc;
    HIPCHK(hipSetDevice(ctx->device));
    const size_t spp = (size_t)p->samples * 4, npx = (size_t)p->width * p->height;
    const size_t n1 = spp * rayn_sets_1d(p->max_bounces, p->volume_marches), n2 = spp * 2 * rayn_sets_2d(p->max_bounces, p->volume_marches);
    const size_t total = n1 + n2 + npx + RAYN_FIS_TABLE_SIZE + npx * RAYN_FILM_FLOATS_PER_PIXEL;
    rc = ensure(ctx, &ctx->host_stage, &ctx->host_stage_cap, total);
    if (rc) return rc;
    float* d = ctx->host_stage;
    float *d1 = d, *d2 = d1 + n1, *dscr = d2 + n2, *dfis = dscr + npx, *dc = dfis + RAYN_FIS_TABLE_SIZE, *da = dc + 3 * npx, *db = da + npx, *dn = db + 3 * npx;
    hipError_t e = hipSuccess;
    auto up = [&](float* dst, const float* src, size_t n) { if (e == hipSuccess) e = hipMemcpyAsync(dst, src, n * 4, hipMemcpyHostToDevice, ctx->stream); };
    up(d1, samples_1d, n1); up(d2, samples_2d, n2); up(dscr, scramble, npx); up(dfis, fis_table, RAYN_FIS_TABLE_SIZE);
    const bool covers = TileGrid(p->width, p->height, p->tile_w, p->tile_h).covers(p->width, p->height, p->tile_w, p->tile_h);
    const bool owns_all = covers && p->tile_step <= 1 && ctx->tile_subset.empty();
    if (!owns_all) { up(dc, out_color, 3 * npx); up(da, out_alpha, npx); up(db, out_background, 3 * npx); up(dn, out_normal, 3 * npx); }
    if (e == hipSuccess) e = hipStreamSynchronize(ctx->stream);
    if (e != hipSuccess) return fail(ctx, RAYN_ERR_HIP, std::string("upload: ") + hipGetErrorString(e));
    rc = render_any(ctx, p, d1, d2, dscr, dfis, RenderTarget{dc, da, db, dn}, ctx->stream);
    if (rc == RAYN_OK) {
        auto down = [&](float* dst, const float* src, size_t n) { if (e == hipSuccess) e = hipMemcpy(dst, src, n * 4, hipMemcpyDeviceToHost); };
        down(out_color, dc, 3 * npx); down(out_alpha, da, npx); down(out_background, db, 3 * npx); down(out_normal, dn, 3 * npx);
        if (e != hipSuccess) rc = fail(ctx, RAYN_ERR_HIP, std::string("download: ") + hipGetErrorString(e));
    }
    return rc;
}

int rayn_hip_get_stats(const rayn_ctx* ctx, rayn_stats* out) {
    if (!ctx || !out) return RAYN_ERR_INVALID_ARG;
    *out = ctx->stats;
    return RAYN_OK;
}

int rayn_hip_set_profiling(rayn_ctx* ctx, int timing, int count_evals) {
    if (!ctx) return RAYN_ERR_INVALID_ARG;
    ctx->cfg->profiling = timing != 0;
    ctx->cfg->counting = count_evals != 0;
    return RAYN_OK;
}
static int get_counts(const rayn_ctx* ctx, const unsigned long long* counts, int n, uint64_t* out) {
    if (!ctx || !out) return RAYN_ERR_INVALID_ARG;
    for (int i = 0; i < n; i++) out[i] = counts[i];
    return RAYN_OK;
}
int rayn_hip_get_eval_counts(const rayn_ctx* ctx, uint64_t out[3]) { return get_counts(ctx, ctx ? ctx->counters.evals : nullptr, 3, out); }
int rayn_hip_get_sdf_iterations(const rayn_ctx* ctx, uint64_t out[3]) { return get_counts(ctx, ctx ? ctx->counters.iters : nullptr, 3, out); }
int rayn_hip_get_elision_counts(const rayn_ctx* ctx, uint64_t out[3]) { return get_counts(ctx, ctx ? ctx->counters.elided : nullptr, 3, out); }
int rayn_hip_get_stage_slots(const rayn_ctx* ctx, uint64_t out[2]) { return get_counts(ctx, ctx ? ctx->counters.stage_slots : nullptr, 2, out); }
int rayn_hip_set_batch_paths(rayn_ctx* ctx, uint64_t paths) {
    if (!ctx || paths < 4096) return RAYN_ERR_INVALID_ARG;
    ctx->cfg->batch_paths = (size_t)paths;
    return RAYN_OK;
}

int rayn_hip_set_cold_bytes(rayn_ctx* ctx, uint64_t bytes) {
    if (!ctx) return RAYN_ERR_INVALID_ARG;
    ctx->cfg->cold_bytes = (size_t)bytes;
    return RAYN_OK;
}

int rayn_hip_set_workers(rayn_ctx* ctx, int n_workers, uint64_t min_paths) {
    if (!ctx || n_workers < 1 || n_workers > MAX_WORKERS) return RAYN_ERR_INVALID_ARG;
    ctx->cfg->n_workers = n_workers;
    ctx->cfg->two_worker_min_paths = (size_t)min_paths;
    return RAYN_OK;
}
int rayn_hip_set_tile_subset(rayn_ctx* ctx, const uint32_t* tiles, uint32_t n) {
    if (!ctx || (n && !tiles)) return RAYN_ERR_INVALID_ARG;
    std::vector<uint32_t> v(tiles, tiles + n);
    std::sort(v.begin(), v.end());
    if (std::adjacent_find(v.begin(), v.end()) != v.end()) return fail(ctx, RAYN_ERR_INVALID_ARG, "duplicate tile index in the subset");
    ctx->tile_subset.swap(v);
    return RAYN_OK;
}
int rayn_hip_set_trace_tile(rayn_ctx* ctx, int tile_index) {
    if (!ctx) return RAYN_ERR_INVALID_ARG;
    if (!ctx->peers.empty()) return fail(ctx, RAYN_ERR_INVALID_ARG, "rayn_hip_set_trace_tile is not supported on a multi-device context");
    ctx->trace_tile = tile_index;
    return RAYN_OK;
}
int64_t rayn_hip_get_trace(const rayn_ctx* ctx, uint32_t* out, uint64_t cap_records) {
    if (!ctx) return RAYN_ERR_INVALID_ARG;
    const uint64_t n = ctx->trace.size() / 6;
    if (out) memcpy(out, ctx->trace.data(), (size_t)std::min(n, cap_records) * 24);
    return (int64_t)n;
}
int rayn_hip_fma_policy(void) { return 0; }
#ifndef RAYN_BUILD_VARIANT
#define RAYN_BUILD_VARIANT ""
#endif
const char* rayn_hip_build_variant(void) { return RAYN_BUILD_VARIANT; }
int rayn_hip_set_fma_policy(rayn_ctx* ctx, int policy) {
    if (!ctx || (policy != 0 && policy != 1)) return RAYN_ERR_INVALID_ARG;
    ctx->cfg->fma_policy = policy;
    return RAYN_OK;
}
size_t rayn_hip_sizeof(int which) {
    switch (which) {
    case 0: return sizeof(rayn_world_desc);
    case 1: return sizeof(rayn_frame_params);
    case 2: return sizeof(rayn_stats);
    case 3: return sizeof(rayn_hitable);
    case 4: return sizeof(rayn_material);
    case 5: return sizeof(rayn_light);
    case 6: return sizeof(rayn_camera);
    case 7: return sizeof(rayn_temporal_resample_params);
    case 8: return sizeof(rayn_display_params);
    case 9: return sizeof(rayn_upscale_params);
    case 10: return sizeof(rayn_temporal_upscale_params);
    case 11: return sizeof(rayn_preview_params);
    case 12: return sizeof(rayn_interpolate_params);
    case 13: return sizeof(rayn_interpolate_key);
    default: return 0;
    }
}

}
```

Before: 265.8 Mpath-samples/s.

## Stop Mandelbox SDF marches early once rays leave a proven bounding hull

Host code derives a conservative bounding slab for the Mandelbox SDF, plus a minimum distance bound and a step budget. The march kernel computes each ray's exit parameter from this hull. Rays that start outside and point away are resolved without any marching. Rays inside stop at the hull exit instead of marching on to t_max, which skips SDF evaluations that cannot hit. Counters and a probe are added for validation, and the added per-lane bookkeeping adds some extra ballots and registers.

Result: no change. 266.5 Mpath-samples/s (median of 6 runs) (+0.3%).

```diff
diff --git a/include/rayn_hip.h b/include/rayn_hip.h
--- a/include/rayn_hip.h
+++ b/include/rayn_hip.h
@@ -364,6 +364,7 @@
 int rayn_hip_get_sdf_iterations(const rayn_ctx* ctx, uint64_t out[3]);
 int rayn_hip_get_elision_counts(const rayn_ctx* ctx, uint64_t out[3]);
 int rayn_hip_get_stage_slots(const rayn_ctx* ctx, uint64_t out[2]);
+int rayn_hip_get_hull_exit_counts(const rayn_ctx* ctx, uint64_t out[2]);
 int rayn_hip_set_workers(rayn_ctx* ctx, int n_workers, uint64_t min_paths);
 int rayn_hip_set_batch_paths(rayn_ctx* ctx, uint64_t paths);
 int rayn_hip_set_cold_bytes(rayn_ctx* ctx, uint64_t bytes);
@@ -406,6 +407,7 @@
 int rayn_hip_probe_sdf_dist_as(rayn_ctx* ctx, const rayn_frame_params* p, uint32_t hitable_index, int32_t sdfk,
                                uint32_t fast_div, float t0, const float* pts_xyz, float* out, uint32_t n);
 int rayn_hip_probe_scene_dispatch(rayn_ctx* ctx, const rayn_frame_params* p, int32_t* out);
+int rayn_hip_probe_hull_exit(rayn_ctx* ctx, const rayn_frame_params* p, uint32_t* out_u, float* out_f);
 int rayn_hip_probe_extend(rayn_ctx* ctx, const rayn_frame_params* p, uint32_t depth,
                           const float* org_xyz, const float* dir_xyz, float* out_t,
                           uint32_t* out_obj, uint32_t n);
diff --git a/rayn_amd/_lib.py b/rayn_amd/_lib.py
--- a/rayn_amd/_lib.py
+++ b/rayn_amd/_lib.py
@@ -28,8 +28,8 @@
     "rayn_hip_render_frame_device", "rayn_hip_get_stats", "rayn_sets_1d", "rayn_sets_2d", "rayn_build_rd_tables",
     "rayn_build_scramble", "rayn_build_fis_table", "rayn_build_fis_table_ex", "rayn_tile_count", "rayn_hip_set_profiling", "rayn_hip_get_eval_counts",
     "rayn_hip_set_batch_paths", "rayn_hip_set_cold_bytes", "rayn_hip_set_workers", "rayn_hip_set_tile_subset", "rayn_hip_set_trace_tile", "rayn_hip_get_trace", "rayn_hip_fma_policy", "rayn_hip_set_fma_policy", "rayn_hip_sizeof", "rayn_hip_probe_sdf_dist",
-    "rayn_hip_probe_extend", "rayn_hip_probe_shadow", "rayn_hip_probe_detmath", "rayn_hip_probe_shading", "rayn_hip_probe_queue", "rayn_hip_probe_resolve", "rayn_hip_probe_march_limits", "rayn_hip_probe_shade", "rayn_hip_probe_shade_limits", "rayn_hip_probe_raygen", "rayn_hip_probe_sdf_dist_as", "rayn_hip_probe_scene_dispatch", "rayn_hip_probe_huffman", "rayn_hip_probe_jpeg_transform", "rayn_hip_probe_jpeg_entropy", "rayn_hip_build_variant",
-    "rayn_hip_get_entry_stats", "rayn_hip_get_sdf_iterations", "rayn_hip_get_elision_counts", "rayn_hip_get_stage_slots", "rayn_share_pixels", "rayn_hip_render_frame_packed_device", "rayn_hip_unpack_share_device",
+    "rayn_hip_probe_extend", "rayn_hip_probe_shadow", "rayn_hip_probe_detmath", "rayn_hip_probe_shading", "rayn_hip_probe_queue", "rayn_hip_probe_resolve", "rayn_hip_probe_march_limits", "rayn_hip_probe_shade", "rayn_hip_probe_shade_limits", "rayn_hip_probe_raygen", "rayn_hip_probe_sdf_dist_as", "rayn_hip_probe_scene_dispatch", "rayn_hip_probe_hull_exit", "rayn_hip_probe_huffman", "rayn_hip_probe_jpeg_transform", "rayn_hip_probe_jpeg_entropy", "rayn_hip_build_variant",
+    "rayn_hip_get_entry_stats", "rayn_hip_get_sdf_iterations", "rayn_hip_get_elision_counts", "rayn_hip_get_stage_slots", "rayn_hip_get_hull_exit_counts", "rayn_share_pixels", "rayn_hip_render_frame_packed_device", "rayn_hip_unpack_share_device",
     "rayn_save_to_bpp", "rayn_hip_save_to_pixels_device", "rayn_denoise_scratch_bytes", "rayn_hip_denoise_device",
     "rayn_progressive_seed", "rayn_progressive_state_bytes", "rayn_hip_progressive_reset_device", "rayn_hip_progressive_accumulate_device",
     "rayn_hip_progressive_fetch_active", "rayn_hip_progressive_tile_report",
@@ -174,6 +174,7 @@
         L.rayn_hip_get_sdf_iterations.argtypes = [vp, C.POINTER(C.c_uint64)]
         L.rayn_hip_get_elision_counts.argtypes = [vp, C.POINTER(C.c_uint64)]
         L.rayn_hip_get_stage_slots.argtypes = [vp, C.POINTER(C.c_uint64)]
+        L.rayn_hip_get_hull_exit_counts.argtypes = [vp, C.POINTER(C.c_uint64)]
         L.rayn_hip_set_batch_paths.argtypes = [vp, C.c_uint64]
         L.rayn_hip_set_cold_bytes.argtypes = [vp, C.c_uint64]
         L.rayn_hip_set_workers.argtypes = [vp, C.c_int, C.c_uint64]
@@ -201,6 +202,7 @@
                                             + [fp] * 5 + [up, bp, up, up, up, up, up, fp])
         L.rayn_hip_probe_sdf_dist_as.argtypes = [vp, C.POINTER(_abi.FrameParams), C.c_uint32, C.c_int32, C.c_uint32, C.c_float, fp, fp, C.c_uint32]
         L.rayn_hip_probe_scene_dispatch.argtypes = [vp, C.POINTER(_abi.FrameParams), C.POINTER(C.c_int32)]
+        L.rayn_hip_probe_hull_exit.argtypes = [vp, C.POINTER(_abi.FrameParams), C.POINTER(C.c_uint32), C.POINTER(C.c_float)]
         L.rayn_hip_probe_huffman.argtypes = [vp, C.c_uint32, C.c_uint32, up, up, up]
         L.rayn_hip_probe_jpeg_transform.argtypes = [vp] + [C.c_uint32] * 5 + [vp, vp]
         L.rayn_hip_probe_jpeg_entropy.argtypes = [vp] + [C.c_uint32] * 5 + [vp, C.c_uint32, vp, C.c_size_t]
diff --git a/rayn_amd/context.py b/rayn_amd/context.py
--- a/rayn_amd/context.py
+++ b/rayn_amd/context.py
@@ -343,6 +343,9 @@
     def stage_slots(self):
         return self._counters(self._L.rayn_hip_get_stage_slots, ("shadow_orbit", "shadow_epilogue"))
 
+    def hull_exit_counts(self):
+        return self._counters(self._L.rayn_hip_get_hull_exit_counts, ("evals_past_exit", "rays_past_exit"))
+
     def render_host(self, params, tables, out=None):
         s1, s2, scr, fis = tables
         n = params.width * params.height
@@ -365,6 +368,11 @@
         self._chk(self._L.rayn_hip_probe_scene_dispatch(self.h, C.byref(params), out))
         v = list(out)
         return {"single_sdf": v[0], "sdf_kind": v[1], "bulb": v[2], "anim_spheres": v[3], "fast_div": [x for x in v[4:] if x >= 0]}
+
+    def probe_hull_exit(self, params):
+        u, f = (C.c_uint32 * 3)(), (C.c_float * 2)()
+        self._chk(self._L.rayn_hip_probe_hull_exit(self.h, C.byref(params), u, f))
+        return {"valid": int(u[0]), "on": int(u[1]), "n_exit": int(u[2]), "h_slab": np.float32(f[0]), "o_max": np.float32(f[1])}
 
     def probe_sdf_dist_as(self, params, hitable_index, sdfk, fast_div, pts, t0=0.0, out=None, check=True):
         pts = np.ascontiguousarray(pts, np.float32).reshape(-1, 3)
diff --git a/rayn_amd/csrc/device_core.h b/rayn_amd/csrc/device_core.h
--- a/rayn_amd/csrc/device_core.h
+++ b/rayn_amd/csrc/device_core.h
@@ -169,7 +169,7 @@
     return mult * lerpf(inverse_cdf[idx], inverse_cdf[idx + 1], t);
 }
 
-struct EvalCtr { uint32_t n = 0, it = 0; };
+struct EvalCtr { uint32_t n = 0, it = 0; uint32_t hull_n = 0, hull_rays = 0; };
 
 __device__ __attribute__((noinline)) static float bulb_logf(float m) { return dmf_logf(m); }
 struct BulbOrbit { f3 w; float m, dz; };
@@ -307,6 +307,19 @@
 }
 RD float thr_at(const Thr& th, float t) { return th.constant ? th.k : th.k * t; }
 
+RD float hull_exit_t(f3 o, f3 d, float H, float o_max) {
+    const float inf = __builtin_inff();
+    const bool in_range = __builtin_fabsf(o.x) <= o_max && __builtin_fabsf(o.y) <= o_max && __builtin_fabsf(o.z) <= o_max &&
+                          __builtin_fabsf(d.x) < inf && __builtin_fabsf(d.y) < inf && __builtin_fabsf(d.z) < inf;
+    if (!in_range) return inf;
+    const float fx = d.x != 0.0f ? (__builtin_copysignf(H, d.x) - o.x) / d.x : (__builtin_fabsf(o.x) > H ? -1.0f : inf);
+    const float fy = d.y != 0.0f ? (__builtin_copysignf(H, d.y) - o.y) / d.y : (__builtin_fabsf(o.y) > H ? -1.0f : inf);
+    const float fz = d.z != 0.0f ? (__builtin_copysignf(H, d.z) - o.z) / d.z : (__builtin_fabsf(o.z) > H ? -1.0f : inf);
+    const float fxy = fy < fx ? fy : fx;
+    const float t_exit = fz < fxy ? fz : fxy;
+    return t_exit < 0.0f ? -1.0f : t_exit;
+}
+
 RD f3 sphere_center(const DHitable& h, float t0) { return h.animated ? h.center + h.center_vel * t0 : h.center; }
 
 template <bool COUNT>
diff --git a/rayn_amd/csrc/device_scene.h b/rayn_amd/csrc/device_scene.h
--- a/rayn_amd/csrc/device_scene.h
+++ b/rayn_amd/csrc/device_scene.h
@@ -34,6 +34,7 @@
     uint32_t _pad_a[2];
     uint32_t width, height, spp, max_bounces, vm, max_marches, max_vis_marches, n1, n2;
     float time_start, time_range, detail_scale, t_max, ndc_x, ndc_y;
+    uint32_t hull_valid, hull_on, hull_n_exit; float hull_h, hull_o_max;
 };
 
 struct DTile { uint32_t x0, y0, ew, eh; uint32_t pool_base, n_paths; uint32_t film_base, film_packed; };
diff --git a/rayn_amd/csrc/driver.h b/rayn_amd/csrc/driver.h
--- a/rayn_amd/csrc/driver.h
+++ b/rayn_amd/csrc/driver.h
@@ -27,16 +27,18 @@
     unsigned long long evals[3] = {0, 0, 0};
     unsigned long long iters[3] = {0, 0, 0};
     unsigned long long elided[3] = {0, 0, 0};
+    unsigned long long hull[2] = {0, 0};
     unsigned long long stage_slots[2] = {0, 0};
     void clear() { *this = Counters(); }
     Counters& operator+=(const Counters& o) {
         for (int k = 0; k < 3; k++) { evals[k] += o.evals[k]; iters[k] += o.iters[k]; elided[k] += o.elided[k]; }
-        for (int k = 0; k < 2; k++) stage_slots[k] += o.stage_slots[k];
+        for (int k = 0; k < 2; k++) { stage_slots[k] += o.stage_slots[k]; hull[k] += o.hull[k]; }
         return *this;
     }
     void decode(const unsigned long long h[16]) {
         for (int k = 0; k < 3; k++) { evals[k] = h[k]; iters[k] = h[4 + k]; }
         elided[0] = h[3]; elided[1] = h[7]; elided[2] = h[8];
+        hull[0] = h[9]; hull[1] = h[10];
         stage_slots[0] = h[12]; stage_slots[1] = h[13];
     }
 };
diff --git a/rayn_amd/csrc/hull_exit.h b/rayn_amd/csrc/hull_exit.h
--- /dev/null
+++ b/rayn_amd/csrc/hull_exit.h
@@ -0,0 +1,41 @@
+#pragma once
+#include <math.h>
+#include <stdint.h>
+
+namespace rayn {
+
+struct HullExit {
+    uint32_t valid;
+    float h_proof;
+    float h_slab;
+    float o_max;
+    float dist_min;
+    uint32_t n_exit;
+};
+
+inline double hull_dist_bound(double a, double l, uint32_t n, double m) {
+    const double an = pow(a, (double)(n + 1u));
+    return ((2.0 * l * a - m) + an * (m - 2.0 * l)) / (an - 1.0);
+}
+
+inline HullExit hull_exit_constants(float scale, float box_l, float min_rad_sq, float fixed_rad_sq, float scale_vel, bool moving_center, uint32_t iterations,
+                                    float thr_max, float t_max) {
+    HullExit z = {0u, 0.0f, 0.0f, 0.0f, 0.0f, 0u};
+    if (!(scale < -1.0f) || !(scale >= -16.0f) || !(box_l > 0.0f) || !(box_l <= 1048576.0f) || !(min_rad_sq <= fixed_rad_sq) || !(fixed_rad_sq > 0.0f) ||
+        !(fixed_rad_sq <= 1099511627776.0f) || scale_vel != 0.0f || moving_center || iterations == 0u || iterations > 12u)
+        return z;
+    if (!(t_max > 0.0f) || !(t_max <= 1048576.0f) || !(thr_max >= 0.0f)) return z;
+    const double a = -(double)scale, l = (double)box_l, R = sqrt((double)fixed_rad_sq);
+    const double H0 = fmax(2.0 * l + R, 4.0 * l);
+    HullExit e = z;
+    e.h_proof = nextafterf((float)(H0 * (1.0 + 1.0 / 1024.0)), INFINITY);
+    e.h_slab = nextafterf((float)((double)e.h_proof * (1.0 + 1.0 / 512.0)), INFINITY);
+    e.o_max = (float)((double)e.h_slab * 1024.0);
+    e.dist_min = nextafterf((float)(hull_dist_bound(a, l, iterations, (double)e.h_proof) * (1.0 - 1.0 / 4096.0)), 0.0f);
+    if (!(e.dist_min > 0.0f) || !((double)e.dist_min >= 2.0 * (double)thr_max) || !((double)e.dist_min >= (double)t_max / 8192.0)) return z;
+    e.n_exit = (uint32_t)ceil((double)t_max / ((double)e.dist_min * (1.0 - 1.0 / 1024.0))) + 1u;
+    e.valid = 1u;
+    return e;
+}
+
+}
diff --git a/rayn_amd/csrc/kernels.h b/rayn_amd/csrc/kernels.h
--- a/rayn_amd/csrc/kernels.h
+++ b/rayn_amd/csrc/kernels.h
@@ -97,6 +97,7 @@
     bool fast_path = true;
     bool sdf_templates = true;
     bool box12s = true;
+    bool hull_exit = true;
     int sdf_kind = -1;
     bool bulb_path = true;
     bool bulb = false;
diff --git a/rayn_amd/csrc/kernels.hip b/rayn_amd/csrc/kernels.hip
--- a/rayn_amd/csrc/kernels.hip
+++ b/rayn_amd/csrc/kernels.hip
@@ -166,6 +166,11 @@
     const uint32_t nh = sc.n_hitables, max_marches = sc.max_marches;
     const DHitable h = sc.h[ks];
     const float c0 = 0.00005f * sc.detail_scale, c1 = 0.05f * sc.detail_scale;
+    constexpr bool HULL = !COUNT && SDFK == SDFK_MANDELBOX_12S;
+    const bool hull = (COUNT ? sc.hull_valid : sc.hull_on) != 0u && depth <= MAX_BOUNCES + 8u;
+    const float hull_h = sc.hull_h, hull_o_max = hull ? sc.hull_o_max : -1.0f;
+    const uint32_t n_exit = sc.hull_n_exit;
+    const uint32_t fit_e = max_marches >= n_exit ? max_marches - n_exit : 0u;
     QueueCursor qc;
     uint64_t cm = 0, nm = 0, nanm = 0;
     uint32_t c_P = 0, c_ent = 0, c_ids = 0, e = 0;
@@ -173,6 +178,8 @@
     f3 o = f3{0, 0, 0}, d = f3{0, 0, 0};
     f3 pt = f3{0, 0, 0};
     float c_pre = 0.0f, c_post = 0.0f, t = 0.0f;
+    float c_stop = 0.0f, n_stop = 0.0f;
+    bool c_past = false;
     float c_scale = h.scale, n_scale = h.scale;
     uint32_t n_P = 0, n_ent = 0, n_ids = 0;
     f3 n_o = f3{0, 0, 0}, n_d = f3{0, 0, 0};
@@ -202,6 +209,18 @@
                         n_ids = id | (idp << 8);
                         n_o = n_o - sphere_center(h, t0);
                         n_scale = sdf_scale(h, t0);
+                        if (HULL || COUNT) {
+                            const float hx = hull_exit_t(n_o, n_d, hull_h, hull_o_max);
+                            if (COUNT) n_stop = hx;
+                            else if (hx < 0.0f && 1u + n_exit <= max_marches) {
+                                const bool post = idp != OBJ_NONE && n_post < n_pre;
+                                if (post) id = idp;
+                                pool.geo1[n_P].z = post ? n_post : n_pre;
+                                ((uint8_t*)&pool.geo1[n_P].w)[0] = (uint8_t)id;
+                                ent_obj[n_ent] = (uint8_t)id;
+                                n_P = INVALID;
+                            } else n_stop = hx >= 0.0f && hx < n_pre ? hx : n_pre;
+                        }
                     }
                 }
                 nm |= take & __builtin_amdgcn_ballot_w64(n_P != INVALID);
@@ -211,6 +230,7 @@
         if (lane_of(fm)) {
             o = n_o; d = n_d; c_pre = n_pre; c_post = n_post; c_ids = n_ids; c_P = n_P; c_ent = n_ent; e = 0;
             c_scale = n_scale;
+            if (HULL || COUNT) { c_stop = n_stop; c_past = false; }
             pt = n_o;
         }
         cm |= fm; nm &= ~fm;
@@ -220,14 +240,30 @@
         }
         float dist = 0.0f;
         if (!COUNT) dist = sdf_dist<COUNT, SDFK>(h, pt, evals, c_scale);
-        else if (lane_of(cm)) dist = sdf_dist<COUNT, SDFK>(h, pt, evals, c_scale);
-        const uint64_t stop = (__builtin_amdgcn_ballot_w64(__builtin_fabsf(dist) < fmaxs(c0, c1 * thr_at(th, t))) | __builtin_amdgcn_ballot_w64(t > c_pre) | nanm) & ~fm;
+        else if (lane_of(cm)) {
+            dist = sdf_dist<COUNT, SDFK>(h, pt, evals, c_scale);
+            if ((lane_of(fm) ? 0.0f : t) > c_stop) { evals.hull_n++; evals.hull_rays += c_past ? 0u : 1u; c_past = true; }
+        }
+        const uint64_t gtm = __builtin_amdgcn_ballot_w64(t > (HULL ? c_stop : c_pre));
+        const uint64_t stop = (__builtin_amdgcn_ballot_w64(__builtin_fabsf(dist) < fmaxs(c0, c1 * thr_at(th, t))) | gtm | nanm) & ~fm;
         nanm = (nanm & ~fm) | (__builtin_amdgcn_ballot_w64(dist != dist) & fm);
         const float ts = t + dist;
         const float tg = lane_of(fm) ? dist : ts;
         t = lane_of(stop) ? t : tg;
         e++;
-        const uint64_t fin = (stop | __builtin_amdgcn_ballot_w64(e == max_marches + 1u)) & cm;
+        uint64_t fin = (stop | __builtin_amdgcn_ballot_w64(e == max_marches + 1u)) & cm;
+        if (HULL) {
+            const uint64_t pc = gtm & ~fm & cm;
+            if (pc != 0) {
+                const uint64_t nofit = pc & ~__builtin_amdgcn_ballot_w64(e <= fit_e);
+                if (lane_of(pc & ~nofit)) t = c_pre;
+                if (nofit != 0) {
+                    const uint64_t keep = nofit & ~__builtin_amdgcn_ballot_w64(t > c_pre);
+                    if (lane_of(keep)) { c_stop = c_pre; e--; }
+                    fin &= ~keep;
+                }
+            }
+        }
         if (lane_of(fin)) {
             float closest = c_pre;
             uint32_t id = c_ids & 0xFFu;
diff --git a/rayn_amd/csrc/march_queue.h b/rayn_amd/csrc/march_queue.h
--- a/rayn_amd/csrc/march_queue.h
+++ b/rayn_amd/csrc/march_queue.h
@@ -90,4 +90,5 @@
 template <bool COUNT>
 RD void flush_evals(const EvalCtr& evals, unsigned long long* __restrict__ evals_out) {
     if (COUNT && evals.n) { atomicAdd(evals_out, (unsigned long long)evals.n); atomicAdd(evals_out + 4, (unsigned long long)evals.it); }
+    if (COUNT && evals.hull_n) { atomicAdd(evals_out + 9, (unsigned long long)evals.hull_n); atomicAdd(evals_out + 10, (unsigned long long)evals.hull_rays); }
 }
diff --git a/rayn_amd/csrc/probes.hip b/rayn_amd/csrc/probes.hip
--- a/rayn_amd/csrc/probes.hip
+++ b/rayn_amd/csrc/probes.hip
@@ -127,6 +127,18 @@
     out[0] = scene_march_kernels(ctx, hs, *p, &tun);
     out[1] = tun.sdf_kind; out[2] = tun.bulb ? 1 : 0; out[3] = (int32_t)hs.anim_spheres;
     for (uint32_t i = 0; i < RAYN_MAX_HITABLES; i++) out[4 + i] = i < hs.n_hitables ? (int32_t)hs.h[i].fast_div : -1;
+    return RAYN_OK;
+}
+int rayn_hip_probe_hull_exit(rayn_ctx* ctx, const rayn_frame_params* p, uint32_t* out_u, float* out_f) {
+    int rc = validate(ctx, p);
+    if (rc) return rc;
+    if (!out_u || !out_f) return fail(ctx, RAYN_ERR_INVALID_ARG, "null buffer");
+    HIPCHK(hipSetDevice(ctx->device));
+    DScene hs;
+    rc = build_scene(ctx, ctx->cfg->world, *p, &hs);
+    if (rc) return rc;
+    out_u[0] = hs.hull_valid; out_u[1] = hs.hull_on; out_u[2] = hs.hull_n_exit;
+    out_f[0] = hs.hull_h; out_f[1] = hs.hull_o_max;
     return RAYN_OK;
 }
 int rayn_hip_probe_extend(rayn_ctx* ctx, const rayn_frame_params* p, uint32_t depth, const float* org, const float* dir, float* out_t,
diff --git a/rayn_amd/csrc/rayn_hip.hip b/rayn_amd/csrc/rayn_hip.hip
--- a/rayn_amd/csrc/rayn_hip.hip
+++ b/rayn_amd/csrc/rayn_hip.hip
@@ -13,6 +13,7 @@
 #include "../../include/rayn_hip.h"
 #include "driver.h"
 #include "frame_layout.h"
+#include "hull_exit.h"
 #include "tiles.h"
 #include "save_to.h"
 #include "display.h"
@@ -145,6 +146,16 @@
     s.time_start = p.time_start; s.time_range = p.time_end - p.time_start;
     s.detail_scale = p.sdf_detail_scale; s.t_max = p.world_radius * 2.0f;
     s.ndc_x = 1.0f / (float)p.width; s.ndc_y = 1.0f / (float)p.height;
+    if (s.n_sdf == 1) for (uint32_t i = 0; i < s.n_hitables; i++) {
+        const DHitable& d = s.h[i];
+        if (d.kind != RAYN_HITABLE_TRACED_SDF || d.sdf_kind != RAYN_SDF_MANDELBOX) continue;
+        const float c0 = 0.00005f * s.detail_scale, c1 = 0.05f * s.detail_scale;
+        const float k_max = std::max(s.cam.half_pixel_size, 0.0001f * 2.0f * (float)(MAX_BOUNCES + 8u));
+        const float thr_max = std::max(c0, c1 * k_max * std::max(1.0f, s.t_max));
+        const HullExit he = hull_exit_constants(d.scale, d.box_l, d.min_rad_sq, d.fixed_rad_sq, d.scale_vel, d.animated != 0u, d.iterations, thr_max, s.t_max);
+        s.hull_valid = he.valid; s.hull_on = he.valid && ctx->tun.hull_exit ? 1u : 0u;
+        s.hull_n_exit = he.n_exit; s.hull_h = he.h_slab; s.hull_o_max = he.o_max;
+    }
     return RAYN_OK;
 }
 
@@ -682,6 +693,7 @@
         if (const char* e = getenv("RAYN_HIP_BULB_STEPS")) ctx->tun.bulb_steps = atoi(e) == 2 ? 2u : 1u;
         if (const char* e = getenv("RAYN_HIP_BULB_ORBIT_MIN")) ctx->tun.bulb_orbit_min = (uint32_t)std::max(0, atoi(e));
         if (const char* e = getenv("RAYN_HIP_BOX12S")) ctx->tun.box12s = atoi(e) != 0;
+        if (const char* e = getenv("RAYN_HIP_HULL_EXIT")) ctx->tun.hull_exit = atoi(e) != 0;
         if (const char* e = getenv("RAYN_HIP_BULB_RAYS")) ctx->tun.bulb_rays = (uint32_t)std::min(4, std::max(2, atoi(e)));
         if (const char* e = getenv("RAYN_HIP_BULB_PREFETCH")) ctx->tun.bulb_prefetch_min = (uint32_t)std::max(1, atoi(e));
     }
@@ -1308,6 +1320,7 @@
 int rayn_hip_get_eval_counts(const rayn_ctx* ctx, uint64_t out[3]) { return get_counts(ctx, ctx ? ctx->counters.evals : nullptr, 3, out); }
 int rayn_hip_get_sdf_iterations(const rayn_ctx* ctx, uint64_t out[3]) { return get_counts(ctx, ctx ? ctx->counters.iters : nullptr, 3, out); }
 int rayn_hip_get_elision_counts(const rayn_ctx* ctx, uint64_t out[3]) { return get_counts(ctx, ctx ? ctx->counters.elided : nullptr, 3, out); }
+int rayn_hip_get_hull_exit_counts(const rayn_ctx* ctx, uint64_t out[2]) { return get_counts(ctx, ctx ? ctx->counters.hull : nullptr, 2, out); }
 int rayn_hip_get_stage_slots(const rayn_ctx* ctx, uint64_t out[2]) { return get_counts(ctx, ctx ? ctx->counters.stage_slots : nullptr, 2, out); }
 int rayn_hip_set_batch_paths(rayn_ctx* ctx, uint64_t paths) {
     if (!ctx || paths < 4096) return RAYN_ERR_INVALID_ARG;
```
